# degleris1/CMF.jl

Hardware: NVIDIA B200
Metric: CNMF iterations/sec (higher is better)
Workload: dtype f32

## Files before the change

cmf.jl_b200/csrc/cmf_sm100.cu:

```cuda
#include "../../include/cmf_sm100.h"

#include <cuda_runtime.h>

#include <algorithm>
#include <chrono>
#include <cmath>
#include <cstdio>
#include <cstring>
#include <map>
#include <memory>
#include <mutex>
#include <tuple>
#include <stdexcept>
#include <string>
#include <vector>

#include <type_traits>

#include "kernels_simt.cuh"
#include "kernels_tc.cuh"
#include "kernels_fd.cuh"
#include "kernels_hals.cuh"
#include "comm.h"

namespace {

thread_local std::string g_err;

struct CmfError : std::runtime_error {
    int code;
    CmfError(int c, const std::string &m) : std::runtime_error(m), code(c) {}
};

#define CK(call)                                                                                   \
    do {                                                                                           \
        cudaError_t e__ = (call);                                                                  \
        if (e__ != cudaSuccess)                                                                    \
            throw CmfError(CMF_ERR_CUDA, std::string(#call) + ": " + cudaGetErrorString(e__));     \
    } while (0)

#define REQUIRE(cond, msg)                                                                         \
    do {                                                                                           \
        if (!(cond)) throw CmfError(CMF_ERR_ARG, std::string(msg));                                \
    } while (0)

inline int64_t cdiv(int64_t a, int64_t b) { return (a + b - 1) / b; }

template <typename T>
struct DevBuf {
    T *p = nullptr;
    size_t n = 0;
    DevBuf() = default;
    DevBuf(const DevBuf &) = delete;
    DevBuf &operator=(const DevBuf &) = delete;
    void alloc(size_t count) {
        free();
        n = count;
        if (count) {
            CK(cudaMalloc(&p, count * sizeof(T)));
            CK(cudaMemsetAsync(p, 0, count * sizeof(T), cudaStreamLegacy));
            CK(cudaStreamSynchronize(cudaStreamLegacy));
        }
    }
    void free() {
        if (p) cudaFree(p);
        p = nullptr;
        n = 0;
    }
    ~DevBuf() { free(); }
};

}

struct cmf_ctx {
    int64_t N = 0, T = 0, t0 = 0, t1 = 0, Tl = 0, K = 0, L = 0;
    int dtype = 0, alg = 0, device = 0, engine = 0;
    bool is_first = true, is_last = true;
    cudaStream_t stream = nullptr;
    bool own_stream = false;
    int64_t launches = 0;
    double data_norm = 0.0;
    double data_sumsq_local = 0.0;
    double data_sumsq_global = 0.0;
    int loss_mode = 0;
    bool loss_mode_explicit = false;
    double loss_guard = 0.25;
    int calib_max_interval = 16;
    bool calib_have = false;
    double calib_bias = 0.0, calib_last_err = 0.0;
    int calib_left = 0, calib_interval = 1, calib_fail = 0;
    int64_t n_loss_direct = 0, n_loss_expansion = 0;
    void calib_reset() { calib_have = false; calib_left = 0; calib_interval = 1; calib_fail = 0; numH_dot_valid = false; }
    double pgd_stepW = 5.0, pgd_stepH = 5.0, pgd_cur_loss = 0.0;
    bool numH_valid = false;
    bool numH_dot_valid = false;
    bool gram_valid = false;
    bool have_data = false, have_factors = false;
    int64_t R = 0;
    bool profiling = false;
    struct ProfEv { int which; cudaEvent_t a, b; };
    std::vector<ProfEv> prof_events;
    int prof_open = -1;
    void prof_begin(int which) {
        if (!profiling) return;
        ProfEv e; e.which = which;
        cudaEventCreate(&e.a); cudaEventCreate(&e.b);
        cudaEventRecord(e.a, stream);
        prof_events.push_back(e);
        prof_open = (int)prof_events.size() - 1;
    }
    void prof_end() {
        if (!profiling || prof_open < 0) return;
        cudaEventRecord(prof_events[prof_open].b, stream);
        prof_open = -1;
    }
    void prof_clear() {
        for (auto &e : prof_events) { cudaEventDestroy(e.a); cudaEventDestroy(e.b); }
        prof_events.clear();
    }
    virtual ~cmf_ctx() {
        prof_clear();
        if (ev_a) cudaEventDestroy(ev_a);
        if (ev_b) cudaEventDestroy(ev_b);
        if (comm_stream) cudaStreamDestroy(comm_stream);
    }
    cmf::Comm comm;
    cudaStream_t comm_stream = nullptr;
    cudaEvent_t ev_a = nullptr, ev_b = nullptr;
    struct cmf_multi *multi = nullptr;
    int world() const { return comm.world; }
    int rank() const { return comm.rank; }
    [[noreturn]] static void no_multi() { throw std::runtime_error("this call is not available on a multi-GPU group handle"); }
    virtual void get_data(void *, int) { no_multi(); }
    virtual bool tc_available() { no_multi(); }
    virtual bool fd_available() { no_multi(); }
    virtual void fd_release() { no_multi(); }
    virtual void set_data(const void *, int64_t) { no_multi(); }
    virtual void synth_data(uint64_t, int64_t, int64_t, double, double) { no_multi(); }
    virtual double data_sumsq() { no_multi(); }
    virtual void set_factors(const void *, const void *, int64_t) { no_multi(); }
    virtual void init_rand(uint64_t) { no_multi(); }
    virtual void init_scale_partials(double *) { no_multi(); }
    virtual void scale_factors(double) { no_multi(); }
    virtual void get_factors(void *, void *) { no_multi(); }
    virtual void w_partials() { no_multi(); }
    virtual void w_apply(double, double) { no_multi(); }
    virtual void w_denom_rows(int64_t, int64_t) { no_multi(); }
    virtual void w_update_rows(double, double, int64_t, int64_t) { no_multi(); }
    virtual void w_rows_buffers(void **, void **, int64_t *) { no_multi(); }
    virtual void fd_denomH_prefetch() {}
    virtual void h_update(double, double) { no_multi(); }
    virtual double loss_partial() { no_multi(); }
    virtual int loss_partial_dev() { no_multi(); }
    virtual double *scalars() { no_multi(); }
    virtual void hals_update_motifs(double, double) { no_multi(); }
    virtual double hals_update_feature_maps(double, double) { no_multi(); }
    virtual void hals_h_prepare() { no_multi(); }
    virtual void hals_h_local(void **, void **, int64_t *) { no_multi(); }
    virtual void hals_h_full(void **, void **) { no_multi(); }
    virtual void hals_h_sweep(int full, double, double) { no_multi(); }
    virtual void h_changed() { no_multi(); }
    virtual void fd_layout(int *, int *, int64_t *) { no_multi(); }
    virtual void set_pgd_loss(int, const void *) { no_multi(); }
    virtual void set_pgd_constraints(int, int) { no_multi(); }
    virtual void pgd_update_motifs(double, double) { no_multi(); }
    virtual double pgd_update_feature_maps(double, double) { no_multi(); }
    virtual void exchange_buffer(int, void **, int64_t *, int *) { no_multi(); }
    virtual void halo_buffers(void **, void **, void **, void **, int64_t *) { no_multi(); }
    virtual void prim_conv(void *) { no_multi(); }
    virtual void prim_transconv(const void *, void *) { no_multi(); }
    virtual void prim_corr(const void *, void *) { no_multi(); }
    virtual void prim_resids(void *) { no_multi(); }
    virtual void prim_shift_and_stack(void *) { no_multi(); }
    virtual void batch_set_factors(const void *, const void *) { no_multi(); }
    virtual void batch_get_factors(void *, void *) { no_multi(); }
    virtual void batch_scale_partials(double *) { no_multi(); }
    virtual void batch_scale(const double *) { no_multi(); }
    virtual void batch_loss(double *) { no_multi(); }
    virtual void batch_set_state(const double *, const int *) { no_multi(); }
    virtual void batch_update_motifs() { no_multi(); }
    virtual void batch_update_feature_maps() { no_multi(); }
};

enum { PROF_CONV = 0, PROF_TRANSCONV = 1, PROF_CORR = 2, PROF_SWEEP = 3, PROF_NCLASS = 4 };

namespace {

using namespace cmf;


typedef CUresult (*EncodeTiledFn)(CUtensorMap *, CUtensorMapDataType, cuuint32_t, void *, const cuuint64_t *,
                                  const cuuint64_t *, const cuuint32_t *, const cuuint32_t *, CUtensorMapInterleave,
                                  CUtensorMapSwizzle, CUtensorMapL2promotion, CUtensorMapFloatOOBfill);

EncodeTiledFn encode_tiled_fn() {
    static EncodeTiledFn fn = nullptr;
    if (!fn) {
        void *ptr = nullptr;
        cudaDriverEntryPointQueryResult qres;
        CK(cudaGetDriverEntryPoint("cuTensorMapEncodeTiled", &ptr, cudaEnableDefault, &qres));
        if (qres != cudaDriverEntryPointSuccess || !ptr) throw CmfError(CMF_ERR_CUDA, "cuTensorMapEncodeTiled not available");
        fn = (EncodeTiledFn)ptr;
    }
    return fn;
}

CUtensorMap make_map_2d(void *base, uint64_t dim0, uint64_t dim1, uint64_t stride1, uint32_t box0, uint32_t box1,
                        CUtensorMapSwizzle swz) {
    CUtensorMap m;
    cuuint64_t gdim[2] = {dim0, dim1};
    cuuint64_t gstr[1] = {stride1};
    cuuint32_t box[2] = {box0, box1};
    cuuint32_t estr[2] = {1, 1};
    CUresult r = encode_tiled_fn()(&m, CU_TENSOR_MAP_DATA_TYPE_BFLOAT16, 2, base, gdim, gstr, box, estr,
                                   CU_TENSOR_MAP_INTERLEAVE_NONE, swz, CU_TENSOR_MAP_L2_PROMOTION_L2_256B,
                                   CU_TENSOR_MAP_FLOAT_OOB_FILL_NONE);
    if (r != CUDA_SUCCESS) throw CmfError(CMF_ERR_CUDA, "cuTensorMapEncodeTiled failed with code " + std::to_string((int)r));
    return m;
}

CUtensorMap make_map_mn(void *base, uint64_t rows, uint64_t row_stride, uint64_t groups, uint32_t box_rows, uint32_t box_groups) {
    CUtensorMap m;
    cuuint64_t gdim[3] = {64, rows, groups};
    cuuint64_t gstr[2] = {row_stride, 128};
    cuuint32_t box[3] = {64, box_rows, box_groups};
    cuuint32_t estr[3] = {1, 1, 1};
    CUresult r = encode_tiled_fn()(&m, CU_TENSOR_MAP_DATA_TYPE_BFLOAT16, 3, base, gdim, gstr, box, estr,
                                   CU_TENSOR_MAP_INTERLEAVE_NONE, CU_TENSOR_MAP_SWIZZLE_128B, CU_TENSOR_MAP_L2_PROMOTION_L2_256B,
                                   CU_TENSOR_MAP_FLOAT_OOB_FILL_NONE);
    if (r != CUDA_SUCCESS) throw CmfError(CMF_ERR_CUDA, "cuTensorMapEncodeTiled (3-D) failed with code " + std::to_string((int)r));
    return m;
}

struct TcState {
    bool ok = false, tried = false;
    int Kp = 0, G = 0, num_sms = 148;
    int64_t KLp = 0, rows_u = 0, groups = 0, hrows = 0;
    DevBuf<__nv_bfloat16> X_hi, X_lo, Hw_hi, Hw_lo, Hm_hi, Hm_lo, Wc_hi, Wc_lo, Wu_hi, Wu_lo, Cc_hi, Cc_lo;
    CUtensorMap mWc[2], mHw[2], mHm[2], mWu[2], mXk[2], mXmn[2];
    CUtensorMap mHmn[2];
    CUtensorMap mCu[2];
    CUtensorMap mHk[2];
    CUtensorMap mGc[2];
    CUtensorMap mWuB[2], mWcB[2];
    DevBuf<__nv_bfloat16> Gc_hi, Gc_lo;
    int nsplit = 1, nsplit_g = 1;
    int64_t split_len = 0, split_len_g = 0, tiles_m = 0, tiles_n = 0, groups_c = 0, rows_c = 0;
    bool x_dirty = true, w_dirty = true;
};

struct FdState {
    bool ok = false, tried = false;
    int B = 0, logB = 0, V = 0, F = 0;
    int64_t nblk = 0, nblkp = 0;
    int Kq = 64, MR = 128;
    int V2 = 0;
    int64_t nblk2 = 0;
    DevBuf<__nv_bfloat16> Xf_hi, Xf_lo, Ah_hi, Ah_lo, Aw_hi, Aw_lo, Hf_hi, Hf_lo, Ac_hi, Ac_lo;
    DevBuf<float> Of, Df, Gf, Yf;
    DevBuf<__nv_bfloat16> Awm_hi, Awm_lo;
    int64_t nbc = 0;
    bool wx_dirty = true;
    CUtensorMap mXfK[2], mXfMN[2], mAw[2], mAh[2], mHfMN[2], mAc[2], mHf2K[2], mAwm[2], mHcK[2];
    bool x_dirty = true, w_dirty = true, h_dirty = true;
    bool hf2_valid = false;
    std::string why;
    void release() {
        Xf_hi.free(); Xf_lo.free(); Ah_hi.free(); Ah_lo.free(); Aw_hi.free(); Aw_lo.free(); Of.free(); Df.free();
        Hf_hi.free(); Hf_lo.free(); Gf.free(); Ac_hi.free(); Ac_lo.free();
        Yf.free(); Awm_hi.free(); Awm_lo.free(); nbc = 0; wx_dirty = true;
        ok = tried = false;
        x_dirty = w_dirty = h_dirty = true; hf2_valid = false;
    }
};

template <typename S>
struct Ctx : cmf_ctx {
    TcState tcs;
    FdState fds;
    DevBuf<S> X, Hbuf, Wi, Wtmp, numW, denW, GS, Cf, numH, denH, tailC;
    DevBuf<int> progress, lockstep;
    DevBuf<S> tailCt;
    int hals_grid = 0;
    DevBuf<double> exch1, corr_part, loss_part, scal;
    S *H = nullptr;
    int nsplit_w = 1, nsplit_g = 1;
    int64_t split_w = 0, split_g = 0;
    int conv_blocks_max = 0;

    static constexpr int TN = sizeof(S) == 4 ? 8 : 4;
    static constexpr int TT = 8, TY = 16;
    static constexpr int BN = 16 * TN, BT = TY * TT;

    int64_t KL() const { return K * L; }

    void hals_setup() {
        REQUIRE(L - 1 <= HW_TC, "HALS: L-1 must not exceed the sweep chunk (1024 columns)");
        const size_t smem = hals_wave_smem_elems<S>(L) * sizeof(S);
        int per_sm = 0, sms = 0, coop = 0;
        CK(cudaDeviceGetAttribute(&sms, cudaDevAttrMultiProcessorCount, device));
        CK(cudaDeviceGetAttribute(&coop, cudaDevAttrCooperativeLaunch, device));
        REQUIRE(coop != 0, "HALS needs cooperative launch support");
        CK(cudaFuncSetAttribute(hals_h_wave_kernel<S>, cudaFuncAttributeMaxDynamicSharedMemorySize, (int)smem));
        CK(cudaOccupancyMaxActiveBlocksPerMultiprocessor(&per_sm, hals_h_wave_kernel<S>, HW_NT, smem));
        hals_grid = (int)std::min<int64_t>(K, (int64_t)per_sm * sms);
        REQUIRE(hals_grid >= 1, "HALS: H sweep kernel does not fit on the device");
        tailC.alloc((size_t)hals_grid * (size_t)(L * L));
        progress.alloc((size_t)K);
    }

    void init() {
        if (R > 0) { init_batch(); return; }
        CK(cudaSetDevice(device));
        CK(cudaStreamCreateWithFlags(&stream, cudaStreamNonBlocking));
        own_stream = true;
        const int64_t hal = L - 1;
        X.alloc((size_t)((Tl + hal) * N));
        Hbuf.alloc((size_t)((Tl + 2 * hal) * K));
        H = Hbuf.p + hal * K;
        Wi.alloc((size_t)(KL() * N));
        Wtmp.alloc((size_t)(KL() * N));
        numW.alloc((size_t)(KL() * N));
        denW.alloc((size_t)(KL() * N));
        GS.alloc((size_t)(KL() * KL()));
        Cf.alloc((size_t)((2 * L - 1) * K * K));
        numH.alloc((size_t)(Tl * K));
        denH.alloc((size_t)(std::max<int64_t>(Tl * K, Tl)));
        exch1.alloc((size_t)(L * K * K + hal * K + 1));
        scal.alloc(8);
        if (alg == CMF_HALS) hals_setup();
        plan_split(N, Tl + hal, nsplit_w, split_w);
        plan_split(K, Tl + hal, nsplit_g, split_g);
        corr_part.alloc((size_t)std::max<int64_t>((int64_t)nsplit_w * KL() * N, (int64_t)nsplit_g * KL() * K));
        conv_blocks_max = (int)(cdiv(N, BN) * cdiv(Tl + hal, BT));
        loss_part.alloc((size_t)std::max(2 * conv_blocks_max, 4096));
        if (sizeof(S) == 4 && N >= 256 && Tl >= 4096 && K * L >= 256) {
            tc_setup();
            const char *e = getenv("CMF_ENGINE_DEFAULT");
            if (tcs.ok && engine == 1 && L >= 8 && K <= fd::KQ_MAX && !(e && atoi(e) == 1)) {
                fd_setup();
                if (fds.ok) { engine = 2; loss_mode = 1; }
            }
        }
        CK(cudaStreamSynchronize(stream));
    }

    bool tc_active() const { return engine >= 1 && tcs.ok; }
    bool fd_active() const { return engine == 2 && tcs.ok && fds.ok; }
    bool fd_available() override {
        if (!tc_available()) return false;
        if (!fds.ok && !fds.tried) fd_setup();
        if (fds.ok) { tcs.X_hi.free(); tcs.X_lo.free(); tcs.x_dirty = true; }
        return fds.ok;
    }
    void fd_release() override { fds.release(); }
    void fd_layout(int *B, int *V, int64_t *nblk) override {
        *B = fd_active() ? fds.B : 0; *V = fd_active() ? fds.V : 0; *nblk = fd_active() ? fds.nblkp : 0;
    }
    void mark_w_dirty() { tcs.w_dirty = true; fds.w_dirty = true; fds.wx_dirty = true; }

    void fd_setup() {
        if constexpr (!std::is_same<S, float>::value) { return; } else {
            FdState &f = fds;
            f.tried = true;
            if (!tcs.ok) { f.why = "needs the tcgen05 engine"; return; }
            if (K > fd::KQ_MAX || L > 256 || N < 16) { f.why = "needs K <= 128, L <= 256, N >= 16"; return; }
            f.Kq = (K <= 64) ? 64 : 128;
            f.MR = 2 * f.Kq;
            int B0 = 64;
            while (B0 < 8 * L && B0 < 1024) B0 *= 2;
            while (B0 < 4 * L) B0 *= 2;
            if (B0 / 2 >= 4 * L && B0 / 2 >= 64) {
                auto work = [&](int B) {
                    const int64_t nb = cdiv(Tl, (int64_t)(B - (int)L + 1));
                    return (double)(B / 2 + 1) * (double)(cdiv(nb, tc::BN) * tc::BN + cdiv(nb, 16) * 16);
                };
                if (work(B0) > 0.97 * work(B0 / 2)) B0 /= 2;
            }
            int forced = 0;
            if (const char *e = getenv("CMF_FD_B")) {
                const int want = atoi(e);
                if (want >= 4 * L && want >= 64 && want <= 1024 && (want & (want - 1)) == 0) forced = want;
            }
            tcs.X_hi.free(); tcs.X_lo.free(); tcs.x_dirty = true;
            size_t free_b = 0, total_b = 0;
            CK(cudaMemGetInfo(&free_b, &total_b));
            size_t later = (size_t)1 << 30;
            if (alg == CMF_HALS) later += (size_t)2 * (size_t)(Tl + 2048) * (size_t)K * 4 + (size_t)hals2::RING * (size_t)cdiv(K, hals2::GS) * (size_t)K * hals2::CW * 4;
            size_t xf = 0, ah = 0, aw = 0, of = 0, df = 0, hf = 0, gf = 0, ac = 0;
            bool fits = false;
            for (int B = forced ? forced : B0; B <= (forced ? forced : std::min(2 * B0, 1024)); B *= 2) {
                int logB = 0;
                while ((1 << logB) < B) ++logB;
                f.B = B; f.logB = logB; f.V = B - (int)L + 1; f.F = B / 2 + 1;
                f.nblk = cdiv(Tl, f.V);
                f.nblkp = cdiv(f.nblk, 16) * 16;
                xf = (size_t)f.F * (size_t)f.nblkp * 2 * (size_t)N + 64;
                ah = (size_t)f.F * (size_t)f.nblkp * 2 * f.MR + 64;
                aw = (size_t)f.F * f.MR * 2 * (size_t)N + 64;
                f.V2 = B - 2 * (int)L + 2;
                f.nblk2 = cdiv(Tl, f.V2);
                of = (size_t)f.F * (size_t)std::max(f.nblkp, f.nblk2) * f.MR; df = (size_t)f.F * f.MR * (size_t)N;
                hf = (size_t)f.F * (size_t)std::max(f.nblkp, f.nblk2) * 2 * f.Kq + 256; gf = (size_t)f.F * f.MR * f.Kq;
                ac = (size_t)f.F * f.MR * f.MR;
                const size_t need = 4 * (xf + ah + aw + hf + ac) + 4 * (of + df + gf);
                const size_t loss_pass = 4 * aw + (size_t)256 * (size_t)f.F * 2 * (size_t)N * sizeof(float);
                if (need + later + loss_pass <= free_b) { fits = true; break; }
            }
            if (!fits) { f.why = "not enough device memory for the spectrum of X"; return; }
            f.Xf_hi.alloc(xf); f.Xf_lo.alloc(xf);
            f.Ah_hi.alloc(ah); f.Ah_lo.alloc(ah);
            f.Aw_hi.alloc(aw); f.Aw_lo.alloc(aw);
            f.Of.alloc(of); f.Df.alloc(df);
            f.Hf_hi.alloc(hf); f.Hf_lo.alloc(hf); f.Gf.alloc(gf);
            f.Ac_hi.alloc(ac); f.Ac_lo.alloc(ac);
            __nv_bfloat16 *xs[2] = {f.Xf_hi.p, f.Xf_lo.p}, *as[2] = {f.Ah_hi.p, f.Ah_lo.p}, *ws[2] = {f.Aw_hi.p, f.Aw_lo.p};
            const uint64_t rows = (uint64_t)f.F * (uint64_t)f.nblkp;
            for (int i = 0; i < 2; ++i) {
                f.mXfK[i] = make_map_2d(xs[i], (uint64_t)(2 * N), rows, (uint64_t)N * 4, tc::BK, tc::BN, CU_TENSOR_MAP_SWIZZLE_64B);
                f.mXfMN[i] = make_map_mn(xs[i], rows * 2, (uint64_t)N * 2, (uint64_t)cdiv(N, 64), tc::BK, 4);
                f.mAw[i] = make_map_2d(ws[i], (uint64_t)(2 * N), (uint64_t)f.F * f.MR, (uint64_t)N * 4, tc::BK, tc::BM, CU_TENSOR_MAP_SWIZZLE_64B);
                f.mAh[i] = make_map_mn(as[i], rows * 2, (uint64_t)f.MR * 2, (uint64_t)(f.MR / 64), tc::BK, 2);
                f.mHfMN[i] = make_map_mn(i == 0 ? f.Hf_hi.p : f.Hf_lo.p, rows * 2, (uint64_t)f.Kq * 2, (uint64_t)(f.Kq / 64), tc::BK, 4);
                f.mAc[i] = make_map_2d(i == 0 ? f.Ac_hi.p : f.Ac_lo.p, f.MR, (uint64_t)f.F * f.MR, (uint64_t)f.MR * 2, tc::BK, tc::BM, CU_TENSOR_MAP_SWIZZLE_64B);
                f.mHf2K[i] = make_map_2d(i == 0 ? f.Hf_hi.p : f.Hf_lo.p, f.MR, (uint64_t)f.F * (uint64_t)f.nblk2, (uint64_t)f.MR * 2, tc::BK, tc::BN, CU_TENSOR_MAP_SWIZZLE_64B);
            }
            CK(cudaFuncSetAttribute(tc::tc_kernel<tc::TC_FQT>, cudaFuncAttributeMaxDynamicSharedMemorySize, tc::SMEM_BYTES));
            CK(cudaFuncSetAttribute(tc::tc_kernel<tc::TC_FQC>, cudaFuncAttributeMaxDynamicSharedMemorySize, tc::SMEM_BYTES));
            CK(cudaFuncSetAttribute(tc::tc_kernel<tc::TC_FQX>, cudaFuncAttributeMaxDynamicSharedMemorySize, tc::SMEM_BYTES));

            const int big = (int)fd_smem(fd_cols_h()), small_ = (int)fd_smem(16);
            CK(cudaFuncSetAttribute(fd::fft_x_kernel, cudaFuncAttributeMaxDynamicSharedMemorySize, small_));
            CK(cudaFuncSetAttribute(fd::ifft_resid_kernel, cudaFuncAttributeMaxDynamicSharedMemorySize, small_));
            CK(cudaFuncSetAttribute(fd::fft_w_kernel, cudaFuncAttributeMaxDynamicSharedMemorySize, small_));
            CK(cudaFuncSetAttribute(fd::ifft_numW_kernel<float>, cudaFuncAttributeMaxDynamicSharedMemorySize, small_));
            CK(cudaFuncSetAttribute(fd::ifft_numW_kernel<double>, cudaFuncAttributeMaxDynamicSharedMemorySize, small_));
            CK(cudaFuncSetAttribute(fd::fft_h_kernel, cudaFuncAttributeMaxDynamicSharedMemorySize, big));
            CK(cudaFuncSetAttribute(fd::ifft_numH_kernel, cudaFuncAttributeMaxDynamicSharedMemorySize, big));
            f.x_dirty = f.w_dirty = f.h_dirty = true;
            f.ok = true;
        }
    }
    int fd_cols_h() const {
        if (const char *e = getenv("CMF_FD_COLS")) {
            const int c = atoi(e);
            if ((c == 8 || c == 16 || c == 32) && (size_t)fds.B * (size_t)c * sizeof(float2) <= 160 * 1024) return c;
        }
        return fds.B >= 1024 ? 8 : 16;
    }
    int64_t fd_order(int64_t nblocks) const { static const int o = getenv("CMF_FD_ORDER") ? atoi(getenv("CMF_FD_ORDER")) : 0; return o ? nblocks : 0; }
    int fd_cols_w() const { return fds.B >= 1024 ? 8 : 16; }
    size_t fd_smem(int C) const { return ((size_t)fds.B * (size_t)C + (size_t)fds.B) * sizeof(float2); }

    void fd_build_X() {
        if constexpr (std::is_same<S, float>::value) {
            FdState &f = fds;
            if (!f.x_dirty) return;
            dim3 grid((unsigned)(f.nblkp * cdiv(N, 32)));
            fd::fft_x_kernel<<<grid, fd::NT, fd_smem(16), stream>>>(X.p, f.Xf_hi.p, f.Xf_lo.p, N, Tl + (L - 1), f.B, f.logB, f.V, f.nblkp, fd_order(f.nblkp));
            post_launch();
            f.x_dirty = false;
        }
    }
    void fd_corr() {
        if constexpr (std::is_same<S, float>::value) {
            FdState &f = fds;
            fd_build_X();
            fd_spectrum_H();
            tc::Params q = tc_base_params();
            q.nprod = 3;
            q.tiles_n = cdiv(N, tc::BN);
            q.nkb = f.nblkp * 2 / tc::BK;
            q.MR = f.MR; q.mtiles = f.MR / tc::BM; q.units = (int64_t)f.F * q.tiles_n * q.mtiles;
            q.fq_rows = f.nblkp * 2;
            q.out = f.Df.p; q.Mrows = f.MR; q.Ncols = N; q.ldo = N;
            const unsigned grid = (unsigned)std::min<int64_t>(q.units, tcs.num_sms);
            prof_begin(PROF_CORR);
            tc::tc_kernel<tc::TC_FQC><<<grid, tc::THREADS, tc::SMEM_BYTES, stream>>>(f.mAh[0], f.mAh[1], f.mXfMN[0], f.mXfMN[1], q);
            prof_end();
            post_launch();
            fd::ifft_numW_kernel<float><<<dim3((unsigned)cdiv(N, 2 * fd_cols_w()), (unsigned)K), fd::NT, fd_smem(fd_cols_w()), stream>>>(f.Df.p, numW.p, N, N, K, L, f.B, f.logB, f.Kq, fd_cols_w());
            post_launch();
        }
    }
    void fd_denomH() {
        if constexpr (std::is_same<S, float>::value) {
            FdState &f = fds;
            fd::fft_w_kernel<<<dim3((unsigned)cdiv(K, 2 * fd_cols_w()), (unsigned)K), fd::NT, fd_smem(fd_cols_w()), stream>>>(
                Cf.p, f.Ac_hi.p, f.Ac_lo.p, K, K, 2 * L - 1, f.B, f.logB, f.MR, f.Kq, 0, f.Kq, fd_cols_w());
            post_launch();
            const int C = fd_cols_h();
            fd_denomH_prefetch();
            f.hf2_valid = false;
            tc::Params q = tc_base_params();
            q.nprod = 3;
            q.tiles_n = cdiv(f.nblk2, tc::BN);
            q.nkb = f.MR / tc::BK;
            q.MR = f.MR; q.mtiles = f.MR / tc::BM; q.units = (int64_t)f.F * q.tiles_n * q.mtiles;
            q.fq_rows = f.nblk2;
            q.out = f.Of.p;
            const unsigned grid = (unsigned)std::min<int64_t>(q.units, tcs.num_sms);
            tc::tc_kernel<tc::TC_FQT><<<grid, tc::THREADS, tc::SMEM_BYTES, stream>>>(f.mAc[0], f.mAc[1], f.mHf2K[0], f.mHf2K[1], q);
            post_launch();
            fd::ifft_numH_kernel<<<(unsigned)(f.nblk2 * (f.Kq / 2 / C)), fd::NT, fd_smem(C), stream>>>(
                f.Of.p, denH.p, K, Tl, f.B, f.logB, f.V2, f.nblk2, C, f.Kq, fd_order(f.nblk2));
            post_launch();
        }
    }
    void fd_denomH_prefetch() override {
        if constexpr (std::is_same<S, float>::value) {
            FdState &f = fds;
            if (!fd_active() || f.hf2_valid) return;
            const int C = fd_cols_h();
            fd::fft_h_kernel<<<(unsigned)(f.nblk2 * (f.Kq / 2 / C)), fd::NT, fd_smem(C), stream>>>(
                H, f.Hf_hi.p, f.Hf_lo.p, K, Tl, Tl + (L - 1), f.B, f.logB, f.V2, f.nblk2, C, 1, -(L - 1), f.Kq, fd_order(f.nblk2));
            post_launch();
            f.hf2_valid = true;
        }
    }
    int64_t fd_conv_loss() {
        if constexpr (std::is_same<S, float>::value) {
            FdState &f = fds;
            f.hf2_valid = false;
            const int64_t ntile32 = cdiv(N, 32);
            if (f.Awm_hi.n == 0) {
                const size_t aw = (size_t)f.F * 2 * f.MR * (size_t)N + 64;
                size_t free_b = 0, total_b = 0;
                CK(cudaMemGetInfo(&free_b, &total_b));
                const size_t per_block = (size_t)f.F * 2 * (size_t)N * sizeof(float);
                REQUIRE(free_b > 4 * aw + 256 * per_block + ((size_t)1 << 29), "not enough device memory for the frequency-domain loss pass");
                size_t budget = std::min<size_t>((free_b - 4 * aw - ((size_t)1 << 29)) / 2, (size_t)12 << 30);
                int64_t nbc = (int64_t)(budget / per_block) / tc::BN * tc::BN;
                nbc = std::max<int64_t>(tc::BN, std::min<int64_t>(nbc, cdiv(f.nblk, tc::BN) * tc::BN));
                if (const char *e = getenv("CMF_FD_NBC")) { const int64_t v = atoll(e); if (v >= tc::BN && v % tc::BN == 0 && v < nbc) nbc = v; }
                f.nbc = nbc;
                f.Awm_hi.alloc(aw); f.Awm_lo.alloc(aw);
                f.Yf.alloc((size_t)f.F * (size_t)nbc * 2 * (size_t)N);
                for (int i = 0; i < 2; ++i) {
                    f.mAwm[i] = make_map_mn(i == 0 ? f.Awm_hi.p : f.Awm_lo.p, (uint64_t)f.F * 2 * f.MR, (uint64_t)N * 2, (uint64_t)cdiv(N, 64), tc::BK, 2);
                    f.mHcK[i] = make_map_2d(i == 0 ? f.Hf_hi.p : f.Hf_lo.p, f.MR, (uint64_t)f.F * (uint64_t)f.nblk, (uint64_t)f.MR * 2, tc::BK, tc::BN, CU_TENSOR_MAP_SWIZZLE_64B);
                }
                f.wx_dirty = true;
            }
            const size_t need_lp = (size_t)(f.nblk * ntile32);
            if (loss_part.n < need_lp) loss_part.alloc(std::max<size_t>(need_lp, 4096));
            if (f.wx_dirty) {
                fd::fft_w_kernel<<<dim3((unsigned)cdiv(N, 2 * fd_cols_w()), (unsigned)K), fd::NT, fd_smem(fd_cols_w()), stream>>>(Wi.p, f.Awm_hi.p, f.Awm_lo.p, N, K, L, f.B, f.logB, 2 * N, N, 1, f.Kq, fd_cols_w());
                post_launch();
                f.wx_dirty = false;
            }
            const int C = fd_cols_h();
            fd::fft_h_kernel<<<(unsigned)(f.nblk * (f.Kq / 2 / C)), fd::NT, fd_smem(C), stream>>>(
                H, f.Hf_hi.p, f.Hf_lo.p, K, Tl, Tl + (L - 1), f.B, f.logB, f.V, f.nblk, C, 1, -(L - 1), f.Kq, fd_order(f.nblk));
            post_launch();
            prof_begin(PROF_CONV);
            for (int64_t b0 = 0; b0 < f.nblk; b0 += f.nbc) {
                const int64_t cur = std::min(f.nbc, f.nblk - b0);
                tc::Params q = tc_base_params();
                q.nprod = 3;
                q.tiles_n = cdiv(cur, tc::BN);
                q.tiles_m = cdiv(N, tc::BM);
                q.nkb = f.MR / tc::BK;
                q.MR = f.MR; q.mtiles = 1; q.units = (int64_t)f.F * 2 * q.tiles_m * q.tiles_n;
                q.fq_rows = f.nblk; q.b_off = b0; q.nbc = cur;
                q.out = f.Yf.p;
                const unsigned grid = (unsigned)std::min<int64_t>(q.units, tcs.num_sms);
                tc::tc_kernel<tc::TC_FQX><<<grid, tc::THREADS, tc::SMEM_BYTES, stream>>>(f.mAwm[0], f.mAwm[1], f.mHcK[0], f.mHcK[1], q);
                post_launch();
                fd::ifft_resid_kernel<<<(unsigned)(cur * ntile32), fd::NT, fd_smem(16), stream>>>(
                    f.Yf.p, X.p, loss_part.p + b0 * ntile32, N, Tl, L, f.B, f.logB, f.V, cur, b0, fd_order(cur));
                post_launch();
            }
            prof_end();
            return f.nblk * ntile32;
        }
        return 0;
    }
    void fd_spectrum_H() {
        if constexpr (std::is_same<S, float>::value) {
            FdState &f = fds;
            if (!f.h_dirty) return;
            const int C = fd_cols_h();
            fd::fft_h_kernel<<<(unsigned)(f.nblkp * (f.Kq / 2 / C)), fd::NT, fd_smem(C), stream>>>(
                H, f.Ah_hi.p, f.Ah_lo.p, K, Tl, Tl + (L - 1), f.B, f.logB, f.V, f.nblkp, C, 0, 0, f.Kq, fd_order(f.nblkp));
            post_launch();
            f.h_dirty = false;
        }
    }
    void fd_gram() {
        if constexpr (std::is_same<S, float>::value) {
            FdState &f = fds;
            f.hf2_valid = false;
            fd_spectrum_H();
            const int C = fd_cols_h();
            fd::fft_h_kernel<<<(unsigned)(f.nblkp * (f.Kq / 2 / C)), fd::NT, fd_smem(C), stream>>>(
                H, f.Hf_hi.p, f.Hf_lo.p, K, Tl, Tl + (L - 1), f.B, f.logB, f.V, f.nblkp, C, 1, 0, f.Kq, fd_order(f.nblkp));
            post_launch();
            tc::Params q = tc_base_params();
            q.nprod = 3;
            q.tiles_n = 1;
            q.nkb = f.nblkp * 2 / tc::BK;
            q.MR = f.MR; q.mtiles = f.MR / tc::BM; q.units = (int64_t)f.F * q.mtiles;
            q.fq_rows = f.nblkp * 2;
            q.out = f.Gf.p; q.Mrows = f.MR; q.Ncols = K; q.ldo = f.Kq;
            const unsigned grid = (unsigned)std::min<int64_t>(q.units, tcs.num_sms);
            tc::tc_kernel<tc::TC_FQC><<<grid, tc::THREADS, tc::SMEM_BYTES, stream>>>(f.mAh[0], f.mAh[1], f.mHfMN[0], f.mHfMN[1], q);
            post_launch();
            fd::ifft_numW_kernel<double><<<dim3((unsigned)cdiv(K, 2 * fd_cols_w()), (unsigned)K), fd::NT, fd_smem(fd_cols_w()), stream>>>(f.Gf.p, exch1.p, K, f.Kq, K, L, f.B, f.logB, f.Kq, fd_cols_w());
            post_launch();
        }
    }
    void fd_transconv() {
        if constexpr (std::is_same<S, float>::value) {
            FdState &f = fds;
            fd_build_X();
            if (f.w_dirty) {
                fd::fft_w_kernel<<<dim3((unsigned)cdiv(N, 2 * fd_cols_w()), (unsigned)K), fd::NT, fd_smem(fd_cols_w()), stream>>>(Wi.p, f.Aw_hi.p, f.Aw_lo.p, N, K, L, f.B, f.logB, 2 * N, N, 0, f.Kq, fd_cols_w());
                post_launch();
                f.w_dirty = false;
            }
            tc::Params q = tc_base_params();
            q.nprod = 3;
            q.tiles_n = cdiv(f.nblkp, tc::BN);
            q.nkb = cdiv(2 * N, tc::BK);
            q.MR = f.MR; q.mtiles = f.MR / tc::BM; q.units = (int64_t)f.F * q.tiles_n * q.mtiles;
            q.fq_rows = f.nblkp;
            q.out = f.Of.p;
            const unsigned grid = (unsigned)std::min<int64_t>(q.units, tcs.num_sms);
            prof_begin(PROF_TRANSCONV);
            tc::tc_kernel<tc::TC_FQT><<<grid, tc::THREADS, tc::SMEM_BYTES, stream>>>(f.mAw[0], f.mAw[1], f.mXfK[0], f.mXfK[1], q);
            prof_end();
            post_launch();
            const int C = fd_cols_h();
            fd::ifft_numH_kernel<<<(unsigned)(f.nblk * (f.Kq / 2 / C)), fd::NT, fd_smem(C), stream>>>(
                f.Of.p, numH.p, K, Tl, f.B, f.logB, f.V, f.nblkp, C, f.Kq, fd_order(f.nblk));
            post_launch();
        }
    }
    bool tc_available() override {
        if (!tcs.ok && !tcs.tried) tc_setup();
        return tcs.ok;
    }

    void tc_setup() {
        if constexpr (!std::is_same<S, float>::value) { return; } else {
            TcState &t = tcs;
            t.tried = true;
            if (K > 128 || N % 8 != 0) return;
            t.Kp = (int)(cdiv(K, 8) * 8);
            t.G = 128 / t.Kp;
            t.KLp = cdiv(L * t.Kp, 64) * 64;
            t.groups = cdiv(L, t.G);
            t.rows_u = cdiv(L * t.Kp + 128, 128) * 128;
            const int64_t hal = L - 1;
            t.hrows = Tl + hal;
            cudaDeviceProp prop;
            CK(cudaGetDeviceProperties(&prop, device));
            if (prop.major != 10) return;
            t.num_sms = prop.multiProcessorCount;
            t.Wc_hi.alloc((size_t)(N * t.KLp)); t.Wc_lo.alloc((size_t)(N * t.KLp));
            t.Wu_hi.alloc((size_t)(t.rows_u * N)); t.Wu_lo.alloc((size_t)(t.rows_u * N));
            t.groups_c = cdiv(2 * L - 1, t.G);
            t.rows_c = cdiv((2 * L - 1) * t.Kp + 128, 128) * 128;
            t.Cc_hi.alloc((size_t)(t.rows_c * t.Kp)); t.Cc_lo.alloc((size_t)(t.rows_c * t.Kp));
            t.Gc_hi.alloc((size_t)(KL() * t.KLp)); t.Gc_lo.alloc((size_t)(KL() * t.KLp));
            if (GS.n < (size_t)(t.rows_u * t.rows_u)) GS.alloc((size_t)(t.rows_u * t.rows_u));
            __nv_bfloat16 *wc[2] = {t.Wc_hi.p, t.Wc_lo.p};
            __nv_bfloat16 *wu[2] = {t.Wu_hi.p, t.Wu_lo.p};
            for (int i = 0; i < 2; ++i) {
                t.mWc[i] = make_map_2d(wc[i], (uint64_t)t.KLp, (uint64_t)N, (uint64_t)t.KLp * 2, tc::BK, tc::BM, CU_TENSOR_MAP_SWIZZLE_64B);
                t.mWu[i] = make_map_2d(wu[i], (uint64_t)N, (uint64_t)t.rows_u, (uint64_t)N * 2, tc::BK, tc::BM, CU_TENSOR_MAP_SWIZZLE_64B);
                __nv_bfloat16 *cc[2] = {t.Cc_hi.p, t.Cc_lo.p};
                t.mCu[i] = make_map_2d(cc[i], (uint64_t)t.Kp, (uint64_t)t.rows_c, (uint64_t)t.Kp * 2, tc::BK, tc::BM, CU_TENSOR_MAP_SWIZZLE_64B);
                __nv_bfloat16 *gc[2] = {t.Gc_hi.p, t.Gc_lo.p};
                t.mWuB[i] = make_map_2d(wu[i], (uint64_t)N, (uint64_t)t.rows_u, (uint64_t)N * 2, tc::BK, tc::BN, CU_TENSOR_MAP_SWIZZLE_64B);
                t.mWcB[i] = make_map_2d(wc[i], (uint64_t)t.KLp, (uint64_t)N, (uint64_t)t.KLp * 2, tc::BK, tc::BN, CU_TENSOR_MAP_SWIZZLE_64B);
                t.mGc[i] = make_map_2d(gc[i], (uint64_t)t.KLp, (uint64_t)KL(), (uint64_t)t.KLp * 2, tc::BK, tc::BM, CU_TENSOR_MAP_SWIZZLE_64B);
            }
            t.tiles_m = cdiv(t.KLp, tc::BM);
            t.tiles_n = cdiv(N, tc::BN);
            const int64_t tau = Tl + hal, base = t.tiles_m * t.tiles_n;
            double best = -1.0;
            for (int ns = 1; ns <= 16; ++ns) {
                const int64_t sl = cdiv(cdiv(tau, ns), tc::BK) * tc::BK;
                if (ns > 1 && sl < tc::FLUSH_T) break;
                const int64_t units = base * cdiv(tau, sl);
                const double eff = (double)units / (double)(cdiv(units, t.num_sms) * t.num_sms);
                if (eff > best + 1e-9) { best = eff; t.nsplit = (int)cdiv(tau, sl); t.split_len = sl; }
            }
            {
                const int64_t want = std::max<int64_t>(1, cdiv(2 * t.num_sms, t.tiles_m));
                const int64_t maxs = std::max<int64_t>(1, tau / tc::FLUSH_T);
                const int64_t ns = std::min(want, maxs);
                t.split_len_g = cdiv(cdiv(tau, ns), tc::BK) * tc::BK;
                t.nsplit_g = (int)cdiv(tau, t.split_len_g);
            }
            const size_t need = std::max((size_t)t.nsplit * (size_t)(KL() * N), (size_t)t.nsplit_g * (size_t)(KL() * K));
            if (corr_part.n < need) corr_part.alloc(need);
            const size_t need_lp = (size_t)(tc::EPI_WARPS * cdiv(Tl, tc::BN) * cdiv(N, tc::BM));
            if (loss_part.n < need_lp) loss_part.alloc(std::max<size_t>(need_lp, 4096));
            CK(cudaFuncSetAttribute(tc::tc_kernel<tc::TC_CONV>, cudaFuncAttributeMaxDynamicSharedMemorySize, tc::SMEM_BYTES));
            CK(cudaFuncSetAttribute(tc::tc_kernel<tc::TC_TRANS>, cudaFuncAttributeMaxDynamicSharedMemorySize, tc::SMEM_BYTES));
            CK(cudaFuncSetAttribute(tc::tc_kernel<tc::TC_CORR>, cudaFuncAttributeMaxDynamicSharedMemorySize, tc::SMEM_BYTES));
            CK(cudaFuncSetAttribute(tc::tc_kernel<tc::TC_PLAIN>, cudaFuncAttributeMaxDynamicSharedMemorySize, tc::SMEM_BYTES));
            t.ok = true;
            t.x_dirty = t.w_dirty = true;
            if (N >= 256 && Tl >= 4096 && K * L >= 256) engine = 1;
        }
    }

    tc::Params tc_base_params() {
        tc::Params q;
        memset(&q, 0, sizeof(q));
        q.N = N; q.K = K; q.L = L; q.Tl = Tl; q.G = tcs.G; q.Kp = tcs.Kp;
        { const char *e = getenv("CMF_PROMO"); q.promo = e ? std::max(1, atoi(e)) : tc::PROMO; }
        { const char *e = getenv("CMF_TC_PRODUCTS"); q.nprod = (e && atoi(e) == 2) ? 2 : 3; }
        return q;
    }

    void tc_split_X() {
        if constexpr (std::is_same<S, float>::value) {
            if (!tcs.ok || !tcs.x_dirty) return;
            TcState &t = tcs;
            if (t.X_hi.n == 0) {
                const int64_t hal = L - 1;
                t.X_hi.alloc(X.n + 64); t.X_lo.alloc(X.n + 64);
                __nv_bfloat16 *xs[2] = {t.X_hi.p, t.X_lo.p};
                for (int i = 0; i < 2; ++i) {
                    t.mXk[i] = make_map_2d(xs[i], (uint64_t)N, (uint64_t)(Tl + hal), (uint64_t)N * 2, tc::BK, tc::BN, CU_TENSOR_MAP_SWIZZLE_64B);
                    t.mXmn[i] = make_map_mn(xs[i], (uint64_t)(Tl + hal), (uint64_t)N * 2, (uint64_t)cdiv(N, 64), tc::BK, 4);
                }
            }
            tc::split_plain_kernel<<<(unsigned)cdiv((int64_t)X.n, 256), 256, 0, stream>>>(X.p, tcs.X_hi.p, tcs.X_lo.p, (int64_t)X.n);
            post_launch();
            tcs.x_dirty = false;
        }
    }
    void tc_split_W() {
        if constexpr (std::is_same<S, float>::value) {
            if (!tcs.w_dirty) return;
            tc::split_W_kernel<<<dim3((unsigned)cdiv(N, 32), (unsigned)cdiv(tcs.Kp, 32), (unsigned)L), dim3(32, 8), 0, stream>>>(
                Wi.p, tcs.Wc_hi.p, tcs.Wc_lo.p, tcs.Wu_hi.p, tcs.Wu_lo.p, N, K, L, tcs.Kp, tcs.KLp);
            post_launch();
            tcs.w_dirty = false;
        }
    }
    void tc_h_planes() {
        if constexpr (std::is_same<S, float>::value) {
            TcState &t = tcs;
            if (t.Hw_hi.n != 0) return;
            const int64_t hal = L - 1;
            const size_t hw_elems = (size_t)((Tl + 2 * hal) * t.Kp + t.KLp + 64);
            t.Hw_hi.alloc(hw_elems); t.Hw_lo.alloc(hw_elems);
            t.Hm_hi.alloc(hw_elems); t.Hm_lo.alloc(hw_elems);
            __nv_bfloat16 *hw[2] = {t.Hw_hi.p, t.Hw_lo.p}, *hm[2] = {t.Hm_hi.p, t.Hm_lo.p};
            for (int i = 0; i < 2; ++i) {
                t.mHw[i] = make_map_2d(hw[i], (uint64_t)t.KLp, (uint64_t)t.hrows, (uint64_t)t.Kp * 2, tc::BK, tc::BN, CU_TENSOR_MAP_SWIZZLE_64B);
                t.mHm[i] = make_map_mn(hm[i], (uint64_t)t.hrows, (uint64_t)t.Kp * 2, (uint64_t)(t.KLp / 64), tc::BK, 2);
                t.mHmn[i] = make_map_mn(hw[i] + hal * t.Kp, (uint64_t)(Tl + hal), (uint64_t)t.Kp * 2, (uint64_t)cdiv(t.Kp, 64), tc::BK, 4);
                t.mHk[i] = make_map_2d(hw[i], (uint64_t)t.Kp, (uint64_t)(Tl + 2 * hal), (uint64_t)t.Kp * 2, tc::BK, tc::BN, CU_TENSOR_MAP_SWIZZLE_64B);
            }
        }
    }
    void tc_split_H(bool masked) {
        if constexpr (std::is_same<S, float>::value) {
            tc_h_planes();
            const int64_t rows = Tl + 2 * (L - 1);
            tc::split_H_kernel<<<(unsigned)cdiv(rows * tcs.Kp, 256), 256, 0, stream>>>(
                Hbuf.p, masked ? tcs.Hm_hi.p : tcs.Hw_hi.p, masked ? tcs.Hm_lo.p : tcs.Hw_lo.p, rows, K, tcs.Kp,
                L - 1, L - 1 + Tl, masked ? 1 : 0);
            post_launch();
        }
    }

    void tc_corr() {
        if constexpr (std::is_same<S, float>::value) {
            if (fd_active()) { fd_corr(); return; }
            tc_split_X();
            tc_split_H(true);
            tc::Params q = tc_base_params();
            q.tiles_m = tcs.tiles_m; q.tiles_n = tcs.tiles_n; q.split_len = tcs.split_len; q.tau_hi = Tl + (L - 1);
            q.units = tcs.tiles_m * tcs.tiles_n * tcs.nsplit;
            q.part = corr_part.p;
            q.corr_order = 0;
            {
                const char *e = getenv("CMF_LOCKSTEP");
                const int w = e ? atoi(e) : 256;
                if (w > 0) {
                    if (lockstep.n == 0) lockstep.alloc(1024);
                    CK(cudaMemsetAsync(lockstep.p, 0, lockstep.n * sizeof(int), stream));
                    q.lockstep = lockstep.p; q.lockstep_window = w;
                }
            }
            const unsigned grid = (unsigned)std::min<int64_t>(q.units, tcs.num_sms);
            prof_begin(PROF_CORR);
            if (q.lockstep != nullptr) {
                void *args[] = {&tcs.mHm[0], &tcs.mHm[1], &tcs.mXmn[0], &tcs.mXmn[1], &q};
                CK(cudaLaunchCooperativeKernel((void *)tc::tc_kernel<tc::TC_CORR>, dim3(grid), dim3(tc::THREADS), args, tc::SMEM_BYTES, stream));
            } else {
                tc::tc_kernel<tc::TC_CORR><<<grid, tc::THREADS, tc::SMEM_BYTES, stream>>>(tcs.mHm[0], tcs.mHm[1], tcs.mXmn[0], tcs.mXmn[1], q);
            }
            prof_end();
            post_launch();
            const int64_t n = KL() * N;
            reduce_partials_kernel<S><<<(unsigned)cdiv(n, 256), 256, 0, stream>>>(corr_part.p, tcs.nsplit, n, numW.p, nullptr);
            post_launch();
        }
    }
    void tc_plain(const CUtensorMap *mA, const CUtensorMap *mB, S *out, int64_t Mrows, int64_t Ncols, int64_t Kdim, int64_t ldo, bool sym = false) {
        if constexpr (std::is_same<S, float>::value) {
            tc::Params q = tc_base_params();
            q.sym = (sym && !getenv("CMF_S2_FULL")) ? 1 : 0;
            q.tiles_n = cdiv(Ncols, tc::BN);
            q.nkb = cdiv(Kdim, tc::BK);
            q.units = q.tiles_n * cdiv(Mrows, tc::BM);
            q.out = out; q.Mrows = Mrows; q.Ncols = Ncols; q.ldo = ldo;
            const unsigned grid = (unsigned)std::min<int64_t>(q.units, tcs.num_sms);
            tc::tc_kernel<tc::TC_PLAIN><<<grid, tc::THREADS, tc::SMEM_BYTES, stream>>>(mA[0], mA[1], mB[0], mB[1], q);
            post_launch();
            if (q.sym) {
                tc::mirror_upper_kernel<<<dim3((unsigned)cdiv(Mrows, 256), (unsigned)Mrows), 256, 0, stream>>>(out, Mrows, ldo);
                post_launch();
            }
        }
    }
    void tc_denomW(int64_t j0 = 0, int64_t j1 = -1) {
        if (j1 < 0) j1 = KL();
        if constexpr (std::is_same<S, float>::value) {
            if (getenv("CMF_G_DIRECT"))
                tc::build_G_split_kernel<<<(unsigned)cdiv(KL() * tcs.KLp, 256), 256, 0, stream>>>(
                    exch1.p, exch1.p + L * K * K, tcs.Gc_hi.p, tcs.Gc_lo.p, K, L, tcs.Kp, tcs.KLp);
            else
                tc::build_G_split_diag_kernel<<<(unsigned)cdiv((2 * L - 1) * K * K, 256), 256, 0, stream>>>(
                    exch1.p, exch1.p + L * K * K, tcs.Gc_hi.p, tcs.Gc_lo.p, K, L, tcs.Kp, tcs.KLp);
            post_launch();
            tc_split_W();
            if (j0 == 0 && j1 == KL()) {
                tc_plain(tcs.mGc, tcs.mWcB, denW.p, KL(), N, tcs.KLp, N);
            } else {
                CUtensorMap mg[2];
                __nv_bfloat16 *gc[2] = {tcs.Gc_hi.p, tcs.Gc_lo.p};
                for (int i = 0; i < 2; ++i)
                    mg[i] = make_map_2d(gc[i] + j0 * tcs.KLp, (uint64_t)tcs.KLp, (uint64_t)(j1 - j0), (uint64_t)tcs.KLp * 2, tc::BK, tc::BM, CU_TENSOR_MAP_SWIZZLE_64B);
                tc_plain(mg, tcs.mWcB, denW.p + j0 * N, j1 - j0, N, tcs.KLp, N);
            }
        }
    }
    void tc_gram() {
        if constexpr (std::is_same<S, float>::value) {
            tc::Params q = tc_base_params();
            q.N = K;
            q.tiles_m = tcs.tiles_m; q.tiles_n = 1; q.split_len = tcs.split_len_g; q.tau_hi = Tl + (L - 1);
            q.units = tcs.tiles_m * tcs.nsplit_g;
            q.part = corr_part.p;
            const unsigned grid = (unsigned)std::min<int64_t>(q.units, tcs.num_sms);
            tc::tc_kernel<tc::TC_CORR><<<grid, tc::THREADS, tc::SMEM_BYTES, stream>>>(tcs.mHm[0], tcs.mHm[1], tcs.mHmn[0], tcs.mHmn[1], q);
            post_launch();
            const int64_t n = L * K * K;
            reduce_partials_kernel<S><<<(unsigned)cdiv(n, 256), 256, 0, stream>>>(corr_part.p, tcs.nsplit_g, n, nullptr, exch1.p);
            post_launch();
        }
    }
    void tc_denomH(bool resplit_C = true) {
        if constexpr (std::is_same<S, float>::value) {
            if (resplit_C) {
                tc::split_C_kernel<<<(unsigned)cdiv(tcs.rows_c * tcs.Kp, 256), 256, 0, stream>>>(Cf.p, tcs.Cc_hi.p, tcs.Cc_lo.p, K, 2 * L - 1, tcs.Kp, tcs.rows_c);
                post_launch();
            }
            tc::Params q = tc_base_params();
            q.groups = tcs.groups_c; q.nblocks = cdiv(tcs.Kp, tc::BK); q.own = tc::BN - (tcs.G - 1);
            q.units = cdiv(Tl, q.own);
            q.out = denH.p;
            const unsigned grid = (unsigned)std::min<int64_t>(q.units, tcs.num_sms);
            tc::tc_kernel<tc::TC_TRANS><<<grid, tc::THREADS, tc::SMEM_BYTES, stream>>>(tcs.mCu[0], tcs.mCu[1], tcs.mHk[0], tcs.mHk[1], q);
            post_launch();
        }
    }
    void tc_transconv() {
        if constexpr (std::is_same<S, float>::value) {
            if (fd_active()) { fd_transconv(); return; }
            tc_split_X();
            tc_split_W();
            tc::Params q = tc_base_params();
            q.groups = tcs.groups; q.nblocks = cdiv(N, tc::BK); q.own = tc::BN - (tcs.G - 1);
            q.units = cdiv(Tl, q.own);
            q.out = numH.p;
            const unsigned grid = (unsigned)std::min<int64_t>(q.units, tcs.num_sms);
            {
                const char *e = getenv("CMF_LOCKSTEP_TRANS");
                const int w = e ? atoi(e) : 0;
                if (w > 0 && q.units >= (int64_t)grid) {
                    if (lockstep.n == 0) lockstep.alloc(1024);
                    CK(cudaMemsetAsync(lockstep.p, 0, lockstep.n * sizeof(int), stream));
                    q.lockstep = lockstep.p; q.lockstep_window = w;
                }
            }
            prof_begin(PROF_TRANSCONV);
            if (q.lockstep != nullptr) {
                void *args[] = {&tcs.mWu[0], &tcs.mWu[1], &tcs.mXk[0], &tcs.mXk[1], &q};
                CK(cudaLaunchCooperativeKernel((void *)tc::tc_kernel<tc::TC_TRANS>, dim3(grid), dim3(tc::THREADS), args, tc::SMEM_BYTES, stream));
            } else {
                tc::tc_kernel<tc::TC_TRANS><<<grid, tc::THREADS, tc::SMEM_BYTES, stream>>>(tcs.mWu[0], tcs.mWu[1], tcs.mXk[0], tcs.mXk[1], q);
            }
            prof_end();
            post_launch();
        }
    }
    int64_t tc_conv_loss() {
        if constexpr (std::is_same<S, float>::value) {
            tc_split_W();
            tc_split_H(false);
            tc::Params q = tc_base_params();
            q.tiles_n = cdiv(N, tc::BM);
            q.nkb = tcs.KLp / tc::BK;
            q.units = q.tiles_n * cdiv(Tl, tc::BN);
            q.X = X.p; q.partial = loss_part.p;
            const unsigned grid = (unsigned)std::min<int64_t>(q.units, tcs.num_sms);
            prof_begin(PROF_CONV);
            tc::tc_kernel<tc::TC_CONV><<<grid, tc::THREADS, tc::SMEM_BYTES, stream>>>(tcs.mWc[0], tcs.mWc[1], tcs.mHw[0], tcs.mHw[1], q);
            prof_end();
            post_launch();
            return tc::EPI_WARPS * q.units;
        }
        return 0;
    }

    ~Ctx() override {
        if (tracing) trace_dump();
        if (own_stream && stream) cudaStreamDestroy(stream);
    }

    void plan_split(int64_t Nin, int64_t tau_hi, int &nsplit, int64_t &split_len, int64_t Kc = 0, int64_t nrest = 1) {
        const int64_t ngrp = cdiv(L, 8);
        const int64_t bxy = cdiv(Nin, 128) * cdiv((Kc ? Kc : K) * ngrp, CORR_PB) * nrest;
        int64_t ns = std::min<int64_t>(std::max<int64_t>(cdiv(592, bxy), 1), 64);
        split_len = cdiv(cdiv(tau_hi, ns), CORR_BTAU) * CORR_BTAU;
        if (split_len < CORR_BTAU) split_len = CORR_BTAU;
        nsplit = (int)cdiv(tau_hi, split_len);
// ... 1855 lines not shown
```

cmf.jl_b200/csrc/kernels_fd.cuh:

```cuda
#pragma once
#include <cuda_bf16.h>
#include <cuda_runtime.h>
#include <stdint.h>

namespace cmf {
namespace fd {

#ifndef CMF_FD_MINB
#define CMF_FD_MINB 3
#endif
constexpr int LD_U = 8;
constexpr int NT = 512;
constexpr int KQ_MAX = 128;

__device__ __forceinline__ void make_twiddles(float2 *tw, int B) {
    for (int m = threadIdx.x; m < B; m += NT) {
        float s, c;
        sincospif(-2.0f * (float)m / (float)B, &s, &c);
        tw[m] = make_float2(c, s);
    }
}

__device__ __forceinline__ int rev(int x, int logB) { return (int)(__brev((unsigned)x) >> (32 - logB)); }

__device__ __forceinline__ float2 cmul(float2 a, float2 w) { return make_float2(a.x * w.x - a.y * w.y, a.x * w.y + a.y * w.x); }
__device__ __forceinline__ float2 cadd(float2 a, float2 b) { return make_float2(a.x + b.x, a.y + b.y); }
__device__ __forceinline__ float2 csub(float2 a, float2 b) { return make_float2(a.x - b.x, a.y - b.y); }
template <bool INV> __device__ __forceinline__ float2 mul_mi(float2 a) { return INV ? make_float2(-a.y, a.x) : make_float2(a.y, -a.x); }
template <bool INV> __device__ __forceinline__ float2 mul_w8(float2 a) {
    const float r = 0.70710678118654752f;
    return INV ? make_float2((a.x - a.y) * r, (a.x + a.y) * r) : make_float2((a.x + a.y) * r, (a.y - a.x) * r);
}
template <bool INV> __device__ __forceinline__ float2 mul_w83(float2 a) {
    const float r = 0.70710678118654752f;
    return INV ? make_float2((-a.x - a.y) * r, (a.x - a.y) * r) : make_float2((a.y - a.x) * r, (-a.x - a.y) * r);
}

template <bool INV>
__device__ __forceinline__ void fft_passes(float2 *d, const float2 *tw, int B, int logB, int C) {
    const int c = threadIdx.x % C, j0 = threadIdx.x / C, jstep = NT / C;
    int s = 0;
    for (; s + 2 < logB; s += 3) {
        const int lq = logB - s - 3, q = 1 << lq, qC = q * C;
        for (int j = j0; j < (B >> 3); j += jstep) {
            const int pos = j & (q - 1), g = j >> lq;
            float2 *r = d + ((g << (lq + 3)) + pos) * C + c;
            float2 a0 = r[0], a1 = r[qC], a2 = r[2 * qC], a3 = r[3 * qC], a4 = r[4 * qC], a5 = r[5 * qC], a6 = r[6 * qC], a7 = r[7 * qC];
            float2 t;
            t = csub(a0, a4); a0 = cadd(a0, a4); a4 = t;
            t = csub(a1, a5); a1 = cadd(a1, a5); a5 = mul_w8<INV>(t);
            t = csub(a2, a6); a2 = cadd(a2, a6); a6 = mul_mi<INV>(t);
            t = csub(a3, a7); a3 = cadd(a3, a7); a7 = mul_w83<INV>(t);
            t = csub(a0, a2); a0 = cadd(a0, a2); a2 = t;
            t = csub(a1, a3); a1 = cadd(a1, a3); a3 = mul_mi<INV>(t);
            t = csub(a4, a6); a4 = cadd(a4, a6); a6 = t;
            t = csub(a5, a7); a5 = cadd(a5, a7); a7 = mul_mi<INV>(t);
            t = csub(a0, a1); a0 = cadd(a0, a1); a1 = t;
            t = csub(a2, a3); a2 = cadd(a2, a3); a3 = t;
            t = csub(a4, a5); a4 = cadd(a4, a5); a5 = t;
            t = csub(a6, a7); a6 = cadd(a6, a7); a7 = t;
            if (lq > 0) {
                const int e = pos << s;
                float2 w;
#define CMF_TW(m_, a_) w = tw[(m_) * e]; if (INV) w.y = -w.y; a_ = cmul(a_, w);
                CMF_TW(4, a1) CMF_TW(2, a2) CMF_TW(6, a3) CMF_TW(1, a4) CMF_TW(5, a5) CMF_TW(3, a6) CMF_TW(7, a7)
#undef CMF_TW
            }
            r[0] = a0; r[qC] = a1; r[2 * qC] = a2; r[3 * qC] = a3; r[4 * qC] = a4; r[5 * qC] = a5; r[6 * qC] = a6; r[7 * qC] = a7;
        }
        __syncthreads();
    }
    if (logB - s == 2) {
        for (int j = j0; j < (B >> 2); j += jstep) {
            float2 *r = d + (4 * j) * C + c;
            float2 a0 = r[0], a1 = r[C], a2 = r[2 * C], a3 = r[3 * C], t;
            t = csub(a0, a2); a0 = cadd(a0, a2); a2 = t;
            t = csub(a1, a3); a1 = cadd(a1, a3); a3 = mul_mi<INV>(t);
            r[0] = cadd(a0, a1); r[C] = csub(a0, a1); r[2 * C] = cadd(a2, a3); r[3 * C] = csub(a2, a3);
        }
        __syncthreads();
    } else if (logB - s == 1) {
        for (int j = j0; j < (B >> 1); j += jstep) {
            float2 *r0 = d + (2 * j) * C + c, *r1 = r0 + C;
            const float2 a = *r0, b = *r1;
            *r0 = cadd(a, b);
            *r1 = csub(a, b);
        }
        __syncthreads();
    }
}

__device__ __forceinline__ void unpack_pair(const float2 *d, int f, int B, int logB, int C, int p, float &ar, float &ai, float &br,
                                            float &bi) {
    const float2 z = d[rev(f, logB) * C + p], y = d[rev((B - f) & (B - 1), logB) * C + p];
    ar = 0.5f * (z.x + y.x); ai = 0.5f * (z.y - y.y);
    br = 0.5f * (z.y + y.y); bi = -0.5f * (z.x - y.x);
}

__device__ __forceinline__ void pack_pair(float2 *d, int f, int B, int C, int p, float2 re, float2 im) {
    if (f == 0 || f == B / 2) im = make_float2(0.f, 0.f);
    d[f * C + p] = make_float2(re.x - im.y, im.x + re.y);
    if (f > 0 && f < B / 2) d[(B - f) * C + p] = make_float2(re.x + im.y, re.y - im.x);
}

__device__ __forceinline__ void split2(float a, float b, uint32_t &h, uint32_t &l) {
    const __nv_bfloat162 hh = __floats2bfloat162_rn(a, b);
    const float2 hf = __bfloat1622float2(hh);
    const __nv_bfloat162 ll = __floats2bfloat162_rn(a - hf.x, b - hf.y);
    h = *reinterpret_cast<const uint32_t *>(&hh);
    l = *reinterpret_cast<const uint32_t *>(&ll);
}
__device__ __forceinline__ void store_split2(__nv_bfloat16 *hi, __nv_bfloat16 *lo, int64_t idx, float a, float b) {
    uint32_t h, l;
    split2(a, b, h, l);
    *reinterpret_cast<uint32_t *>(hi + idx) = h;
    *reinterpret_cast<uint32_t *>(lo + idx) = l;
}

__global__ void __launch_bounds__(NT, CMF_FD_MINB)
fft_x_kernel(const float *__restrict__ X, __nv_bfloat16 *__restrict__ hi, __nv_bfloat16 *__restrict__ lo, int64_t N, int64_t xcols,
             int B, int logB, int V, int64_t nblkp, int64_t nbx) {
    extern __shared__ float2 fd_smem[];
    constexpr int C = 16;
    float2 *d = fd_smem, *tw = fd_smem + (size_t)B * C;
    const int ny = (int)((N + 31) / 32);
    const int64_t b = nbx ? blockIdx.x % nbx : blockIdx.x / ny;
    const int p = threadIdx.x % C;
    const int64_t n = (int64_t)(nbx ? blockIdx.x / nbx : blockIdx.x % ny) * 32 + 2 * p;
    make_twiddles(tw, B);
    {
        const int i0 = threadIdx.x / C, istep = NT / C;
        const int64_t lim64 = xcols - b * V;
        const int lim = (n < N) ? (int)(lim64 < 0 ? 0 : (lim64 > B ? B : lim64)) : 0;
        const float *src = X + (b * V + i0) * N + n;
        for (int i = i0; i < B; i += LD_U * istep, src += (int64_t)LD_U * istep * N) {
            float2 v[LD_U];
#pragma unroll
            for (int u = 0; u < LD_U; ++u) {
                v[u] = make_float2(0.f, 0.f);
                if (i + u * istep < lim) v[u] = *reinterpret_cast<const float2 *>(src + (int64_t)u * istep * N);
            }
#pragma unroll
            for (int u = 0; u < LD_U; ++u)
                if (i + u * istep < B) d[(i + u * istep) * C + p] = v[u];
        }
    }
    __syncthreads();
    fft_passes<false>(d, tw, B, logB, C);
    if (n >= N) return;
    for (int f = threadIdx.x / C; f <= B / 2; f += NT / C) {
        float ar, ai, br, bi;
        unpack_pair(d, f, B, logB, C, p, ar, ai, br, bi);
        const int64_t r = ((int64_t)f * nblkp + b) * 2;
        store_split2(hi, lo, r * N + n, ar, br);
        store_split2(hi, lo, (r + 1) * N + n, ai, bi);
    }
}

__global__ void __launch_bounds__(NT, CMF_FD_MINB)
fft_h_kernel(const float *__restrict__ H, __nv_bfloat16 *__restrict__ hi, __nv_bfloat16 *__restrict__ lo, int64_t K, int64_t Tl,
             int64_t hcols, int B, int logB, int V, int64_t nblkp, int C, int full, int64_t t_off, int kq, int64_t nbx) {
    const int64_t KQ = kq, MROWS = 2 * kq;
    extern __shared__ float2 fd_smem[];
    float2 *d = fd_smem, *tw = fd_smem + (size_t)B * C;
    const int ny = (kq / 2) / C;
    const int64_t b = nbx ? blockIdx.x % nbx : blockIdx.x / ny;
    const int p = threadIdx.x % C;
    const int k = 2 * ((int)(nbx ? blockIdx.x / nbx : blockIdx.x % ny) * C + p);
    make_twiddles(tw, B);
    {
        const int i0 = threadIdx.x / C, istep = NT / C;
        const int64_t tb = b * V + t_off;
        const int64_t lim64 = full ? (hcols - tb) : ((Tl - tb < V) ? Tl - tb : V);
        const int lim = (int)(lim64 < 0 ? 0 : (lim64 > B ? B : lim64));
        const float *src = H + (tb + i0) * K + k;
        const bool pair = ((K & 1) == 0) && (k + 1 < K);
        for (int i = i0; i < B; i += LD_U * istep, src += (int64_t)LD_U * istep * K) {
            float2 v[LD_U];
#pragma unroll
            for (int u = 0; u < LD_U; ++u) {
                v[u] = make_float2(0.f, 0.f);
                if (i + u * istep < lim) {
                    const float *q = src + (int64_t)u * istep * K;
                    if (pair) v[u] = *reinterpret_cast<const float2 *>(q);
                    else { if (k < K) v[u].x = q[0]; if (k + 1 < K) v[u].y = q[1]; }
                }
            }
#pragma unroll
            for (int u = 0; u < LD_U; ++u)
                if (i + u * istep < B) d[(i + u * istep) * C + p] = v[u];
        }
    }
    __syncthreads();
    fft_passes<false>(d, tw, B, logB, C);
    for (int f = threadIdx.x / C; f <= B / 2; f += NT / C) {
        float ar, ai, br, bi;
        unpack_pair(d, f, B, logB, C, p, ar, ai, br, bi);
        uint32_t hr, lr, hi_, li_;
        split2(ar, br, hr, lr);
        split2(ai, bi, hi_, li_);
        if (full) {
            const int64_t r = (((int64_t)f * nblkp + b) * 2) * KQ + k;
            *reinterpret_cast<uint32_t *>(hi + r) = hr; *reinterpret_cast<uint32_t *>(lo + r) = lr;
            *reinterpret_cast<uint32_t *>(hi + r + KQ) = hi_; *reinterpret_cast<uint32_t *>(lo + r + KQ) = li_;
            continue;
        }
        const int64_t r = (((int64_t)f * nblkp + b) * 2) * MROWS + k;
        const uint32_t sg = 0x80008000u;
        *reinterpret_cast<uint32_t *>(hi + r) = hr; *reinterpret_cast<uint32_t *>(lo + r) = lr;
        *reinterpret_cast<uint32_t *>(hi + r + KQ) = hi_ ^ sg; *reinterpret_cast<uint32_t *>(lo + r + KQ) = li_ ^ sg;
        *reinterpret_cast<uint32_t *>(hi + r + MROWS) = hi_; *reinterpret_cast<uint32_t *>(lo + r + MROWS) = li_;
        *reinterpret_cast<uint32_t *>(hi + r + MROWS + KQ) = hr; *reinterpret_cast<uint32_t *>(lo + r + MROWS + KQ) = lr;
    }
}

__global__ void __launch_bounds__(NT, CMF_FD_MINB)
fft_w_kernel(const float *__restrict__ Wi, __nv_bfloat16 *__restrict__ hi, __nv_bfloat16 *__restrict__ lo, int64_t N, int64_t K,
             int64_t L, int B, int logB, int64_t ldw, int64_t coff, int xmode, int kq, int C) {
    const int64_t KQ = kq, MROWS = 2 * kq;
    extern __shared__ float2 fd_smem[];
    float2 *d = fd_smem, *tw = fd_smem + (size_t)B * C;
    const int64_t k = blockIdx.y;
    const int p = threadIdx.x % C;
    const int64_t n = (int64_t)blockIdx.x * (2 * C) + 2 * p;
    make_twiddles(tw, B);
    {
        const int i0 = threadIdx.x / C, istep = NT / C;
        for (int i = i0; i < B; i += LD_U * istep) {
            float2 v[LD_U];
#pragma unroll
            for (int u = 0; u < LD_U; ++u) {
                const int ii = i + u * istep;
                v[u] = make_float2(0.f, 0.f);
                if (ii < L && n < N) {
                    const float *src = Wi + ((int64_t)ii * K + k) * N + n;
                    if ((N & 1) == 0) v[u] = *reinterpret_cast<const float2 *>(src);
                    else { v[u].x = src[0]; if (n + 1 < N) v[u].y = src[1]; }
                }
            }
#pragma unroll
            for (int u = 0; u < LD_U; ++u)
                if (i + u * istep < B) d[(i + u * istep) * C + p] = v[u];
        }
    }
    __syncthreads();
    fft_passes<false>(d, tw, B, logB, C);
    if (n >= N) return;
    for (int f = threadIdx.x / C; f <= B / 2; f += NT / C) {
        float ar, ai, br, bi;
        unpack_pair(d, f, B, logB, C, p, ar, ai, br, bi);
        if (xmode) {
            const int64_t r0 = (((int64_t)f * 2 + 0) * MROWS + k) * N + n, r1 = (((int64_t)f * 2 + 1) * MROWS + k) * N + n;
            store_split2(hi, lo, r0, ar, br);
            store_split2(hi, lo, r0 + KQ * N, -ai, -bi);
            store_split2(hi, lo, r1, ai, bi);
            store_split2(hi, lo, r1 + KQ * N, ar, br);
            continue;
        }
        const int64_t re = ((int64_t)f * MROWS + k) * ldw, im = ((int64_t)f * MROWS + KQ + k) * ldw;
        store_split2(hi, lo, re + n, ar, br);
        store_split2(hi, lo, re + coff + n, ai, bi);
        store_split2(hi, lo, im + n, -ai, -bi);
        store_split2(hi, lo, im + coff + n, ar, br);
    }
}

__global__ void __launch_bounds__(NT, CMF_FD_MINB)
ifft_numH_kernel(const float *__restrict__ Of, float *__restrict__ numH, int64_t K, int64_t Tl, int B, int logB, int V,
                 int64_t nblkp, int C, int kq, int64_t nbx) {
    const int64_t KQ = kq, MROWS = 2 * kq;
    extern __shared__ float2 fd_smem[];
    float2 *d = fd_smem, *tw = fd_smem + (size_t)B * C;
    const int ny = (kq / 2) / C;
    const int64_t b = nbx ? blockIdx.x % nbx : blockIdx.x / ny;
    const int p = threadIdx.x % C;
    const int k = 2 * ((int)(nbx ? blockIdx.x / nbx : blockIdx.x % ny) * C + p);
    make_twiddles(tw, B);
    {
        const int f0 = threadIdx.x / C, fstep = NT / C;
        const float *o = Of + ((int64_t)f0 * nblkp + b) * MROWS + k;
        for (int f = f0; f <= B / 2; f += 4 * fstep, o += (int64_t)4 * fstep * nblkp * MROWS) {
            float2 re[4], im[4];
#pragma unroll
            for (int u = 0; u < 4; ++u)
                if (f + u * fstep <= B / 2) {
                    const float *q = o + (int64_t)u * fstep * nblkp * MROWS;
                    re[u] = *reinterpret_cast<const float2 *>(q); im[u] = *reinterpret_cast<const float2 *>(q + KQ);
                }
#pragma unroll
            for (int u = 0; u < 4; ++u)
                if (f + u * fstep <= B / 2) pack_pair(d, f + u * fstep, B, C, p, re[u], im[u]);
        }
    }
    __syncthreads();
    fft_passes<true>(d, tw, B, logB, C);
    const float sc = 1.0f / (float)B;
    const bool pair = ((K & 1) == 0) && (k + 1 < K);
    for (int i = threadIdx.x / C; i < V; i += NT / C) {
        const int64_t t = b * V + i;
        if (t >= Tl) break;
        const float2 z = d[rev(i, logB) * C + p];
        if (pair) *reinterpret_cast<float2 *>(numH + t * K + k) = make_float2(z.x * sc, z.y * sc);
        else { if (k < K) numH[t * K + k] = z.x * sc; if (k + 1 < K) numH[t * K + k + 1] = z.y * sc; }
    }
}

__global__ void __launch_bounds__(NT, CMF_FD_MINB)
ifft_resid_kernel(const float *__restrict__ Yf, const float *__restrict__ X, double *__restrict__ partial, int64_t N, int64_t Tl,
                  int64_t L, int B, int logB, int V, int64_t nbc, int64_t b0, int64_t nbx) {
    extern __shared__ float2 fd_smem[];
    __shared__ double red[NT / 32];
    constexpr int C = 16;
    float2 *d = fd_smem, *tw = fd_smem + (size_t)B * C;
    const int ny = (int)((N + 31) / 32);
    const int64_t bc = nbx ? blockIdx.x % nbx : blockIdx.x / ny;
    const int by = (int)(nbx ? blockIdx.x / nbx : blockIdx.x % ny);
    const int p = threadIdx.x % C;
    const int64_t n = (int64_t)by * 32 + 2 * p;
    make_twiddles(tw, B);
    {
        const int f0 = threadIdx.x / C, fstep = NT / C;
        const float *y = Yf + (((int64_t)f0 * nbc + bc) * 2) * N + n;
        for (int f = f0; f <= B / 2; f += 4 * fstep, y += (int64_t)4 * fstep * nbc * 2 * N) {
            float2 re[4], im[4];
#pragma unroll
            for (int u = 0; u < 4; ++u) {
                re[u] = make_float2(0.f, 0.f); im[u] = re[u];
                if (f + u * fstep <= B / 2 && n < N) {
                    const float *q = y + (int64_t)u * fstep * nbc * 2 * N;
                    re[u] = *reinterpret_cast<const float2 *>(q); im[u] = *reinterpret_cast<const float2 *>(q + N);
                }
            }
#pragma unroll
            for (int u = 0; u < 4; ++u)
                if (f + u * fstep <= B / 2) pack_pair(d, f + u * fstep, B, C, p, re[u], im[u]);
        }
    }
    __syncthreads();
    fft_passes<true>(d, tw, B, logB, C);
    const float sc = 1.0f / (float)B;
    double accd = 0.0;
    if (n < N) {
        const int istep = NT / C;
        const int64_t tb = (b0 + bc) * V - (L - 1);
        for (int i = (int)(L - 1) + threadIdx.x / C; i < B; i += LD_U * istep) {
            float2 x[LD_U];
#pragma unroll
            for (int u = 0; u < LD_U; ++u) {
                const int ii = i + u * istep;
                x[u] = make_float2(0.f, 0.f);
                if (ii < B && tb + ii < Tl) x[u] = *reinterpret_cast<const float2 *>(X + (tb + ii) * N + n);
            }
            float acc = 0.f;
#pragma unroll
            for (int u = 0; u < LD_U; ++u) {
                const int ii = i + u * istep;
                if (ii < B && tb + ii < Tl) {
                    const float2 z = d[rev(ii, logB) * C + p];
                    const float r0 = z.x * sc - x[u].x, r1 = z.y * sc - x[u].y;
                    acc = fmaf(r0, r0, acc);
                    acc = fmaf(r1, r1, acc);
                }
            }
            accd += (double)acc;
        }
    }
#pragma unroll
    for (int o = 16; o > 0; o >>= 1) accd += __shfl_xor_sync(0xffffffffu, accd, o);
    if ((threadIdx.x & 31) == 0) red[threadIdx.x >> 5] = accd;
    __syncthreads();
    if (threadIdx.x == 0) {
        double s = 0.0;
        for (int w = 0; w < NT / 32; ++w) s += red[w];
        partial[bc * ny + by] = s;
    }
}

template <typename OutT>
__global__ void __launch_bounds__(NT, CMF_FD_MINB)
ifft_numW_kernel(const float *__restrict__ Df, OutT *__restrict__ out, int64_t N, int64_t ldi, int64_t K, int64_t L, int B, int logB,
                 int kq, int C) {
    const int64_t KQ = kq, MROWS = 2 * kq;
    extern __shared__ float2 fd_smem[];
    float2 *d = fd_smem, *tw = fd_smem + (size_t)B * C;
    const int64_t k = blockIdx.y;
    const int p = threadIdx.x % C;
    const int64_t n = (int64_t)blockIdx.x * (2 * C) + 2 * p;
    make_twiddles(tw, B);
    {
        const int f0 = threadIdx.x / C, fstep = NT / C;
        for (int f = f0; f <= B / 2; f += 4 * fstep) {
            float2 re[4], im[4];
#pragma unroll
            for (int u = 0; u < 4; ++u) {
                const int ff = f + u * fstep;
                re[u] = make_float2(0.f, 0.f); im[u] = re[u];
                if (ff <= B / 2 && n < N) {
                    re[u] = *reinterpret_cast<const float2 *>(Df + ((int64_t)ff * MROWS + k) * ldi + n);
                    im[u] = *reinterpret_cast<const float2 *>(Df + ((int64_t)ff * MROWS + KQ + k) * ldi + n);
                }
            }
#pragma unroll
            for (int u = 0; u < 4; ++u)
                if (f + u * fstep <= B / 2) pack_pair(d, f + u * fstep, B, C, p, re[u], im[u]);
        }
    }
    __syncthreads();
    fft_passes<true>(d, tw, B, logB, C);
    if (n >= N) return;
    const float sc = 1.0f / (float)B;
    for (int l = threadIdx.x / C; l < L; l += NT / C) {
        const float2 z = d[rev(l, logB) * C + p];
        OutT *o = out + ((int64_t)l * K + k) * N + n;
        if (sizeof(OutT) == 4) {
            *reinterpret_cast<float2 *>(o) = make_float2(z.x * sc, z.y * sc);
        } else {
            o[0] = (OutT)(z.x * sc);
            if (n + 1 < N) o[1] = (OutT)(z.y * sc);
        }
    }
}

}
}
```

Measured before the change: 23.23.

## Template FFT kernels on block length and width, precompute twiddles, use packed float2 math

The frequency-domain FFT kernels become templates on log block length and tile width, so loop bounds, strides and bit-reversal are compile-time constants and loops can be fully unrolled. Twiddle factors are computed once into a device buffer and copied into shared memory, instead of each block evaluating sincospif. The butterfly and scaling arithmetic uses packed float2 intrinsics (__fadd2_rn, __ffma2_rn). In exchange there are many more kernel instantiations, and block lengths outside 64–1024 are rejected.

After: 24.98, median of 6. +7.5%, better.

```diff
diff --git a/cmf.jl_b200/csrc/cmf_sm100.cu b/cmf.jl_b200/csrc/cmf_sm100.cu
--- a/cmf.jl_b200/csrc/cmf_sm100.cu
+++ b/cmf.jl_b200/csrc/cmf_sm100.cu
@@ -258,6 +258,7 @@
     int64_t nblk2 = 0;
     DevBuf<__nv_bfloat16> Xf_hi, Xf_lo, Ah_hi, Ah_lo, Aw_hi, Aw_lo, Hf_hi, Hf_lo, Ac_hi, Ac_lo;
     DevBuf<float> Of, Df, Gf, Yf;
+    DevBuf<float2> tw;
     DevBuf<__nv_bfloat16> Awm_hi, Awm_lo;
     int64_t nbc = 0;
     bool wx_dirty = true;
@@ -267,12 +268,35 @@
     std::string why;
     void release() {
         Xf_hi.free(); Xf_lo.free(); Ah_hi.free(); Ah_lo.free(); Aw_hi.free(); Aw_lo.free(); Of.free(); Df.free();
-        Hf_hi.free(); Hf_lo.free(); Gf.free(); Ac_hi.free(); Ac_lo.free();
+        Hf_hi.free(); Hf_lo.free(); Gf.free(); Ac_hi.free(); Ac_lo.free(); tw.free();
         Yf.free(); Awm_hi.free(); Awm_lo.free(); nbc = 0; wx_dirty = true;
         ok = tried = false;
         x_dirty = w_dirty = h_dirty = true; hf2_valid = false;
     }
 };
+
+template <typename Fn>
+void fd_with_b(int logB, Fn &&fn) {
+    switch (logB) {
+    case 6: fn(std::integral_constant<int, 6>{}); break;
+    case 7: fn(std::integral_constant<int, 7>{}); break;
+    case 8: fn(std::integral_constant<int, 8>{}); break;
+    case 9: fn(std::integral_constant<int, 9>{}); break;
+    case 10: fn(std::integral_constant<int, 10>{}); break;
+    default: REQUIRE(false, "frequency-domain transforms: block length must be a power of two in [64, 1024]");
+    }
+}
+template <typename Fn>
+void fd_with_bc(int logB, int C, Fn &&fn) {
+    fd_with_b(logB, [&](auto lb) {
+        switch (C) {
+        case 8: fn(lb, std::integral_constant<int, 8>{}); break;
+        case 16: fn(lb, std::integral_constant<int, 16>{}); break;
+        case 32: fn(lb, std::integral_constant<int, 32>{}); break;
+        default: REQUIRE(false, "frequency-domain transforms: unsupported tile width");
+        }
+    });
+}
 
 template <typename S>
 struct Ctx : cmf_ctx {
@@ -414,6 +438,9 @@
             f.Of.alloc(of); f.Df.alloc(df);
             f.Hf_hi.alloc(hf); f.Hf_lo.alloc(hf); f.Gf.alloc(gf);
             f.Ac_hi.alloc(ac); f.Ac_lo.alloc(ac);
+            f.tw.alloc((size_t)f.B);
+            fd::twiddle_kernel<<<(unsigned)cdiv(f.B, 256), 256, 0, stream>>>(f.tw.p, f.B);
+            post_launch();
             __nv_bfloat16 *xs[2] = {f.Xf_hi.p, f.Xf_lo.p}, *as[2] = {f.Ah_hi.p, f.Ah_lo.p}, *ws[2] = {f.Aw_hi.p, f.Aw_lo.p};
             const uint64_t rows = (uint64_t)f.F * (uint64_t)f.nblkp;
             for (int i = 0; i < 2; ++i) {
@@ -429,14 +456,27 @@
             CK(cudaFuncSetAttribute(tc::tc_kernel<tc::TC_FQC>, cudaFuncAttributeMaxDynamicSharedMemorySize, tc::SMEM_BYTES));
             CK(cudaFuncSetAttribute(tc::tc_kernel<tc::TC_FQX>, cudaFuncAttributeMaxDynamicSharedMemorySize, tc::SMEM_BYTES));
 
-            const int big = (int)fd_smem(fd_cols_h()), small_ = (int)fd_smem(16);
-            CK(cudaFuncSetAttribute(fd::fft_x_kernel, cudaFuncAttributeMaxDynamicSharedMemorySize, small_));
-            CK(cudaFuncSetAttribute(fd::ifft_resid_kernel, cudaFuncAttributeMaxDynamicSharedMemorySize, small_));
-            CK(cudaFuncSetAttribute(fd::fft_w_kernel, cudaFuncAttributeMaxDynamicSharedMemorySize, small_));
-            CK(cudaFuncSetAttribute(fd::ifft_numW_kernel<float>, cudaFuncAttributeMaxDynamicSharedMemorySize, small_));
-            CK(cudaFuncSetAttribute(fd::ifft_numW_kernel<double>, cudaFuncAttributeMaxDynamicSharedMemorySize, small_));
-            CK(cudaFuncSetAttribute(fd::fft_h_kernel, cudaFuncAttributeMaxDynamicSharedMemorySize, big));
-            CK(cudaFuncSetAttribute(fd::ifft_numH_kernel, cudaFuncAttributeMaxDynamicSharedMemorySize, big));
+            fd_with_b(f.logB, [&](auto lb) {
+                constexpr int LB = decltype(lb)::value;
+                const int x16 = (int)fd_smem(16), w = (int)fd_smem(fd_cols_w());
+                CK(cudaFuncSetAttribute(fd::fft_x_kernel<LB>, cudaFuncAttributeMaxDynamicSharedMemorySize, x16));
+                CK(cudaFuncSetAttribute(fd::ifft_resid_kernel<LB>, cudaFuncAttributeMaxDynamicSharedMemorySize, x16));
+                fd_with_bc(f.logB, fd_cols_w(), [&](auto, auto c) {
+                    constexpr int CW = decltype(c)::value;
+                    CK(cudaFuncSetAttribute(fd::fft_w_kernel<LB, CW>, cudaFuncAttributeMaxDynamicSharedMemorySize, w));
+                    CK(cudaFuncSetAttribute(fd::ifft_numW_kernel<float, LB, CW>, cudaFuncAttributeMaxDynamicSharedMemorySize, w));
+                    CK(cudaFuncSetAttribute(fd::ifft_numW_kernel<double, LB, CW>, cudaFuncAttributeMaxDynamicSharedMemorySize, w));
+                });
+                for (int ch : {8, 16, 32}) {
+                    if (LB == 10 && ch == 32) continue;
+                    const int h = (int)fd_smem(ch);
+                    fd_with_bc(f.logB, ch, [&](auto, auto c) {
+                        constexpr int CH = decltype(c)::value;
+                        CK(cudaFuncSetAttribute(fd::fft_h_kernel<LB, CH>, cudaFuncAttributeMaxDynamicSharedMemorySize, h));
+                        CK(cudaFuncSetAttribute(fd::ifft_numH_kernel<LB, CH>, cudaFuncAttributeMaxDynamicSharedMemorySize, h));
+                    });
+                }
+            });
             f.x_dirty = f.w_dirty = f.h_dirty = true;
             f.ok = true;
         }
@@ -451,13 +491,45 @@
     int64_t fd_order(int64_t nblocks) const { static const int o = getenv("CMF_FD_ORDER") ? atoi(getenv("CMF_FD_ORDER")) : 0; return o ? nblocks : 0; }
     int fd_cols_w() const { return fds.B >= 1024 ? 8 : 16; }
     size_t fd_smem(int C) const { return ((size_t)fds.B * (size_t)C + (size_t)fds.B) * sizeof(float2); }
+    void fd_fft_h(__nv_bfloat16 *hi, __nv_bfloat16 *lo, int64_t nb, int V, int full, int64_t t_off) {
+        const int C = fd_cols_h();
+        fd_with_bc(fds.logB, C, [&](auto lb, auto c) {
+            fd::fft_h_kernel<decltype(lb)::value, decltype(c)::value><<<(unsigned)(nb * (fds.Kq / 2 / C)), fd::NT, fd_smem(C), stream>>>(
+                H, hi, lo, K, Tl, Tl + (L - 1), V, nb, full, t_off, fds.Kq, fd_order(nb), fds.tw.p);
+        });
+    }
+    void fd_ifft_numH(const float *Of, float *out, int64_t nb, int V, int64_t nblkp_) {
+        const int C = fd_cols_h();
+        fd_with_bc(fds.logB, C, [&](auto lb, auto c) {
+            fd::ifft_numH_kernel<decltype(lb)::value, decltype(c)::value><<<(unsigned)(nb * (fds.Kq / 2 / C)), fd::NT, fd_smem(C), stream>>>(
+                Of, out, K, Tl, V, nblkp_, fds.Kq, fd_order(nb), fds.tw.p);
+        });
+    }
+    void fd_fft_w(const float *src, __nv_bfloat16 *hi, __nv_bfloat16 *lo, int64_t Nw, int64_t Lw, int64_t ldw, int64_t coff, int xmode) {
+        const int C = fd_cols_w();
+        fd_with_bc(fds.logB, C, [&](auto lb, auto c) {
+            fd::fft_w_kernel<decltype(lb)::value, decltype(c)::value><<<dim3((unsigned)cdiv(Nw, 2 * C), (unsigned)K), fd::NT, fd_smem(C), stream>>>(
+                src, hi, lo, Nw, K, Lw, ldw, coff, xmode, fds.Kq, fds.tw.p);
+        });
+    }
+    template <typename OutT>
+    void fd_ifft_numW(const float *Df, OutT *out, int64_t Nw, int64_t ldi) {
+        const int C = fd_cols_w();
+        fd_with_bc(fds.logB, C, [&](auto lb, auto c) {
+            fd::ifft_numW_kernel<OutT, decltype(lb)::value, decltype(c)::value><<<dim3((unsigned)cdiv(Nw, 2 * C), (unsigned)K), fd::NT, fd_smem(C), stream>>>(
+                Df, out, Nw, ldi, K, L, fds.Kq, fds.tw.p);
+        });
+    }
 
     void fd_build_X() {
         if constexpr (std::is_same<S, float>::value) {
             FdState &f = fds;
             if (!f.x_dirty) return;
             dim3 grid((unsigned)(f.nblkp * cdiv(N, 32)));
-            fd::fft_x_kernel<<<grid, fd::NT, fd_smem(16), stream>>>(X.p, f.Xf_hi.p, f.Xf_lo.p, N, Tl + (L - 1), f.B, f.logB, f.V, f.nblkp, fd_order(f.nblkp));
+            fd_with_b(f.logB, [&](auto lb) {
+                fd::fft_x_kernel<decltype(lb)::value><<<grid, fd::NT, fd_smem(16), stream>>>(X.p, f.Xf_hi.p, f.Xf_lo.p, N, Tl + (L - 1), f.V, f.nblkp,
+                                                                                            fd_order(f.nblkp), f.tw.p);
+            });
             post_launch();
             f.x_dirty = false;
         }
@@ -479,17 +551,15 @@
             tc::tc_kernel<tc::TC_FQC><<<grid, tc::THREADS, tc::SMEM_BYTES, stream>>>(f.mAh[0], f.mAh[1], f.mXfMN[0], f.mXfMN[1], q);
             prof_end();
             post_launch();
-            fd::ifft_numW_kernel<float><<<dim3((unsigned)cdiv(N, 2 * fd_cols_w()), (unsigned)K), fd::NT, fd_smem(fd_cols_w()), stream>>>(f.Df.p, numW.p, N, N, K, L, f.B, f.logB, f.Kq, fd_cols_w());
+            fd_ifft_numW(f.Df.p, numW.p, N, N);
             post_launch();
         }
     }
     void fd_denomH() {
         if constexpr (std::is_same<S, float>::value) {
             FdState &f = fds;
-            fd::fft_w_kernel<<<dim3((unsigned)cdiv(K, 2 * fd_cols_w()), (unsigned)K), fd::NT, fd_smem(fd_cols_w()), stream>>>(
-                Cf.p, f.Ac_hi.p, f.Ac_lo.p, K, K, 2 * L - 1, f.B, f.logB, f.MR, f.Kq, 0, f.Kq, fd_cols_w());
-            post_launch();
-            const int C = fd_cols_h();
+            fd_fft_w(Cf.p, f.Ac_hi.p, f.Ac_lo.p, K, 2 * L - 1, f.MR, f.Kq, 0);
+            post_launch();
             fd_denomH_prefetch();
             f.hf2_valid = false;
             tc::Params q = tc_base_params();
@@ -502,8 +572,7 @@
             const unsigned grid = (unsigned)std::min<int64_t>(q.units, tcs.num_sms);
             tc::tc_kernel<tc::TC_FQT><<<grid, tc::THREADS, tc::SMEM_BYTES, stream>>>(f.mAc[0], f.mAc[1], f.mHf2K[0], f.mHf2K[1], q);
             post_launch();
-            fd::ifft_numH_kernel<<<(unsigned)(f.nblk2 * (f.Kq / 2 / C)), fd::NT, fd_smem(C), stream>>>(
-                f.Of.p, denH.p, K, Tl, f.B, f.logB, f.V2, f.nblk2, C, f.Kq, fd_order(f.nblk2));
+            fd_ifft_numH(f.Of.p, denH.p, f.nblk2, f.V2, f.nblk2);
             post_launch();
         }
     }
@@ -511,9 +580,7 @@
         if constexpr (std::is_same<S, float>::value) {
             FdState &f = fds;
             if (!fd_active() || f.hf2_valid) return;
-            const int C = fd_cols_h();
-            fd::fft_h_kernel<<<(unsigned)(f.nblk2 * (f.Kq / 2 / C)), fd::NT, fd_smem(C), stream>>>(
-                H, f.Hf_hi.p, f.Hf_lo.p, K, Tl, Tl + (L - 1), f.B, f.logB, f.V2, f.nblk2, C, 1, -(L - 1), f.Kq, fd_order(f.nblk2));
+            fd_fft_h(f.Hf_hi.p, f.Hf_lo.p, f.nblk2, f.V2, 1, -(L - 1));
             post_launch();
             f.hf2_valid = true;
         }
@@ -545,13 +612,11 @@
             const size_t need_lp = (size_t)(f.nblk * ntile32);
             if (loss_part.n < need_lp) loss_part.alloc(std::max<size_t>(need_lp, 4096));
             if (f.wx_dirty) {
-                fd::fft_w_kernel<<<dim3((unsigned)cdiv(N, 2 * fd_cols_w()), (unsigned)K), fd::NT, fd_smem(fd_cols_w()), stream>>>(Wi.p, f.Awm_hi.p, f.Awm_lo.p, N, K, L, f.B, f.logB, 2 * N, N, 1, f.Kq, fd_cols_w());
+                fd_fft_w(Wi.p, f.Awm_hi.p, f.Awm_lo.p, N, L, 2 * N, N, 1);
                 post_launch();
                 f.wx_dirty = false;
             }
-            const int C = fd_cols_h();
-            fd::fft_h_kernel<<<(unsigned)(f.nblk * (f.Kq / 2 / C)), fd::NT, fd_smem(C), stream>>>(
-                H, f.Hf_hi.p, f.Hf_lo.p, K, Tl, Tl + (L - 1), f.B, f.logB, f.V, f.nblk, C, 1, -(L - 1), f.Kq, fd_order(f.nblk));
+            fd_fft_h(f.Hf_hi.p, f.Hf_lo.p, f.nblk, f.V, 1, -(L - 1));
             post_launch();
             prof_begin(PROF_CONV);
             for (int64_t b0 = 0; b0 < f.nblk; b0 += f.nbc) {
@@ -567,8 +632,10 @@
                 const unsigned grid = (unsigned)std::min<int64_t>(q.units, tcs.num_sms);
                 tc::tc_kernel<tc::TC_FQX><<<grid, tc::THREADS, tc::SMEM_BYTES, stream>>>(f.mAwm[0], f.mAwm[1], f.mHcK[0], f.mHcK[1], q);
                 post_launch();
-                fd::ifft_resid_kernel<<<(unsigned)(cur * ntile32), fd::NT, fd_smem(16), stream>>>(
-                    f.Yf.p, X.p, loss_part.p + b0 * ntile32, N, Tl, L, f.B, f.logB, f.V, cur, b0, fd_order(cur));
+                fd_with_b(f.logB, [&](auto lb) {
+                    fd::ifft_resid_kernel<decltype(lb)::value><<<(unsigned)(cur * ntile32), fd::NT, fd_smem(16), stream>>>(
+                        f.Yf.p, X.p, loss_part.p + b0 * ntile32, N, Tl, L, f.V, cur, b0, fd_order(cur), f.tw.p);
+                });
                 post_launch();
             }
             prof_end();
@@ -580,9 +647,7 @@
         if constexpr (std::is_same<S, float>::value) {
             FdState &f = fds;
             if (!f.h_dirty) return;
-            const int C = fd_cols_h();
-            fd::fft_h_kernel<<<(unsigned)(f.nblkp * (f.Kq / 2 / C)), fd::NT, fd_smem(C), stream>>>(
-                H, f.Ah_hi.p, f.Ah_lo.p, K, Tl, Tl + (L - 1), f.B, f.logB, f.V, f.nblkp, C, 0, 0, f.Kq, fd_order(f.nblkp));
+            fd_fft_h(f.Ah_hi.p, f.Ah_lo.p, f.nblkp, f.V, 0, 0);
             post_launch();
             f.h_dirty = false;
         }
@@ -592,9 +657,7 @@
             FdState &f = fds;
             f.hf2_valid = false;
             fd_spectrum_H();
-            const int C = fd_cols_h();
-            fd::fft_h_kernel<<<(unsigned)(f.nblkp * (f.Kq / 2 / C)), fd::NT, fd_smem(C), stream>>>(
-                H, f.Hf_hi.p, f.Hf_lo.p, K, Tl, Tl + (L - 1), f.B, f.logB, f.V, f.nblkp, C, 1, 0, f.Kq, fd_order(f.nblkp));
+            fd_fft_h(f.Hf_hi.p, f.Hf_lo.p, f.nblkp, f.V, 1, 0);
             post_launch();
             tc::Params q = tc_base_params();
             q.nprod = 3;
@@ -606,7 +669,7 @@
             const unsigned grid = (unsigned)std::min<int64_t>(q.units, tcs.num_sms);
             tc::tc_kernel<tc::TC_FQC><<<grid, tc::THREADS, tc::SMEM_BYTES, stream>>>(f.mAh[0], f.mAh[1], f.mHfMN[0], f.mHfMN[1], q);
             post_launch();
-            fd::ifft_numW_kernel<double><<<dim3((unsigned)cdiv(K, 2 * fd_cols_w()), (unsigned)K), fd::NT, fd_smem(fd_cols_w()), stream>>>(f.Gf.p, exch1.p, K, f.Kq, K, L, f.B, f.logB, f.Kq, fd_cols_w());
+            fd_ifft_numW(f.Gf.p, exch1.p, K, f.Kq);
             post_launch();
         }
     }
@@ -615,7 +678,7 @@
             FdState &f = fds;
             fd_build_X();
             if (f.w_dirty) {
-                fd::fft_w_kernel<<<dim3((unsigned)cdiv(N, 2 * fd_cols_w()), (unsigned)K), fd::NT, fd_smem(fd_cols_w()), stream>>>(Wi.p, f.Aw_hi.p, f.Aw_lo.p, N, K, L, f.B, f.logB, 2 * N, N, 0, f.Kq, fd_cols_w());
+                fd_fft_w(Wi.p, f.Aw_hi.p, f.Aw_lo.p, N, L, 2 * N, N, 0);
                 post_launch();
                 f.w_dirty = false;
             }
@@ -631,9 +694,7 @@
             tc::tc_kernel<tc::TC_FQT><<<grid, tc::THREADS, tc::SMEM_BYTES, stream>>>(f.mAw[0], f.mAw[1], f.mXfK[0], f.mXfK[1], q);
             prof_end();
             post_launch();
-            const int C = fd_cols_h();
-            fd::ifft_numH_kernel<<<(unsigned)(f.nblk * (f.Kq / 2 / C)), fd::NT, fd_smem(C), stream>>>(
-                f.Of.p, numH.p, K, Tl, f.B, f.logB, f.V, f.nblkp, C, f.Kq, fd_order(f.nblk));
+            fd_ifft_numH(f.Of.p, numH.p, f.nblk, f.V, f.nblkp);
             post_launch();
         }
     }
diff --git a/cmf.jl_b200/csrc/kernels_fd.cuh b/cmf.jl_b200/csrc/kernels_fd.cuh
--- a/cmf.jl_b200/csrc/kernels_fd.cuh
+++ b/cmf.jl_b200/csrc/kernels_fd.cuh
@@ -13,199 +13,242 @@
 constexpr int NT = 512;
 constexpr int KQ_MAX = 128;
 
-__device__ __forceinline__ void make_twiddles(float2 *tw, int B) {
-    for (int m = threadIdx.x; m < B; m += NT) {
+__device__ __forceinline__ float2 add2(float2 a, float2 b) { return __fadd2_rn(a, b); }
+__device__ __forceinline__ float2 sub2(float2 a, float2 b) { return __fadd2_rn(a, make_float2(-b.x, -b.y)); }
+__device__ __forceinline__ float2 mul2(float2 a, float2 b) { return __fmul2_rn(a, b); }
+__device__ __forceinline__ float2 fma2(float2 a, float2 b, float2 c) { return __ffma2_rn(a, b, c); }
+__device__ __forceinline__ float2 bcast(float x) { return make_float2(x, x); }
+
+__global__ void twiddle_kernel(float2 *__restrict__ tw, int B) {
+    const int m = blockIdx.x * blockDim.x + threadIdx.x;
+    if (m < B) {
         float s, c;
         sincospif(-2.0f * (float)m / (float)B, &s, &c);
         tw[m] = make_float2(c, s);
     }
 }
-
-__device__ __forceinline__ int rev(int x, int logB) { return (int)(__brev((unsigned)x) >> (32 - logB)); }
-
-__device__ __forceinline__ float2 cmul(float2 a, float2 w) { return make_float2(a.x * w.x - a.y * w.y, a.x * w.y + a.y * w.x); }
-__device__ __forceinline__ float2 cadd(float2 a, float2 b) { return make_float2(a.x + b.x, a.y + b.y); }
-__device__ __forceinline__ float2 csub(float2 a, float2 b) { return make_float2(a.x - b.x, a.y - b.y); }
+template <int B>
+__device__ __forceinline__ void load_twiddles(float2 *tw, const float2 *__restrict__ twg) {
+#pragma unroll
+    for (int m = threadIdx.x; m < B; m += NT) tw[m] = twg[m];
+}
+
+__device__ __forceinline__ void grid_block_tile(int64_t nbx, int ny, int &blk, int &tile) {
+    const unsigned dv = nbx ? (unsigned)nbx : (unsigned)ny, q = blockIdx.x / dv, r = blockIdx.x - q * dv;
+    blk = (int)(nbx ? r : q);
+    tile = (int)(nbx ? q : r);
+}
+
+template <int LOGB> __device__ __forceinline__ int rev(int x) { return (int)(__brev((unsigned)x) >> (32 - LOGB)); }
+
+template <bool INV> __device__ __forceinline__ float2 twmul(float2 a, float2 w) {
+    const float2 t = mul2(make_float2(a.y, a.x), INV ? make_float2(w.y, -w.y) : make_float2(-w.y, w.y));
+    return fma2(a, bcast(w.x), t);
+}
 template <bool INV> __device__ __forceinline__ float2 mul_mi(float2 a) { return INV ? make_float2(-a.y, a.x) : make_float2(a.y, -a.x); }
-template <bool INV> __device__ __forceinline__ float2 mul_w8(float2 a) {
-    const float r = 0.70710678118654752f;
-    return INV ? make_float2((a.x - a.y) * r, (a.x + a.y) * r) : make_float2((a.x + a.y) * r, (a.y - a.x) * r);
-}
-template <bool INV> __device__ __forceinline__ float2 mul_w83(float2 a) {
-    const float r = 0.70710678118654752f;
-    return INV ? make_float2((-a.x - a.y) * r, (a.x - a.y) * r) : make_float2((a.y - a.x) * r, (-a.x - a.y) * r);
-}
-
-template <bool INV>
-__device__ __forceinline__ void fft_passes(float2 *d, const float2 *tw, int B, int logB, int C) {
-    const int c = threadIdx.x % C, j0 = threadIdx.x / C, jstep = NT / C;
-    int s = 0;
-    for (; s + 2 < logB; s += 3) {
-        const int lq = logB - s - 3, q = 1 << lq, qC = q * C;
-        for (int j = j0; j < (B >> 3); j += jstep) {
+template <bool INV> __device__ __forceinline__ float2 w8_sum(float2 a) {
+    return INV ? add2(make_float2(a.x, a.x), make_float2(-a.y, a.y)) : add2(a, make_float2(a.y, -a.x));
+}
+template <bool INV> __device__ __forceinline__ float2 w83_sum(float2 a) {
+    return INV ? add2(make_float2(-a.x, a.x), make_float2(-a.y, -a.y)) : add2(make_float2(a.y, -a.x), make_float2(-a.x, -a.y));
+}
+
+template <bool INV, int LOGB, int C>
+__device__ __forceinline__ void fft_passes(float2 *d, const float2 *tw) {
+    constexpr int B = 1 << LOGB, JSTEP = NT / C;
+    const float2 rr = bcast(0.70710678118654752f);
+    const int c = threadIdx.x % C, j0 = threadIdx.x / C;
+#pragma unroll
+    for (int s = 0; s + 2 < LOGB; s += 3) {
+        const int lq = LOGB - s - 3, q = 1 << lq, qC = q * C;
+#pragma unroll 1
+        for (int jj = 0; jj < (B / 8 + JSTEP - 1) / JSTEP; ++jj) {
+            const int j = j0 + jj * JSTEP;
+            if ((B / 8) % JSTEP != 0 && j >= B / 8) break;
             const int pos = j & (q - 1), g = j >> lq;
             float2 *r = d + ((g << (lq + 3)) + pos) * C + c;
             float2 a0 = r[0], a1 = r[qC], a2 = r[2 * qC], a3 = r[3 * qC], a4 = r[4 * qC], a5 = r[5 * qC], a6 = r[6 * qC], a7 = r[7 * qC];
-            float2 t;
-            t = csub(a0, a4); a0 = cadd(a0, a4); a4 = t;
-            t = csub(a1, a5); a1 = cadd(a1, a5); a5 = mul_w8<INV>(t);
-            t = csub(a2, a6); a2 = cadd(a2, a6); a6 = mul_mi<INV>(t);
-            t = csub(a3, a7); a3 = cadd(a3, a7); a7 = mul_w83<INV>(t);
-            t = csub(a0, a2); a0 = cadd(a0, a2); a2 = t;
-            t = csub(a1, a3); a1 = cadd(a1, a3); a3 = mul_mi<INV>(t);
-            t = csub(a4, a6); a4 = cadd(a4, a6); a6 = t;
-            t = csub(a5, a7); a5 = cadd(a5, a7); a7 = mul_mi<INV>(t);
-            t = csub(a0, a1); a0 = cadd(a0, a1); a1 = t;
-            t = csub(a2, a3); a2 = cadd(a2, a3); a3 = t;
-            t = csub(a4, a5); a4 = cadd(a4, a5); a5 = t;
-            t = csub(a6, a7); a6 = cadd(a6, a7); a7 = t;
+            float2 t, u5, v7;
+            t = sub2(a0, a4); a0 = add2(a0, a4); a4 = t;
+            t = sub2(a1, a5); a1 = add2(a1, a5); u5 = w8_sum<INV>(t);
+            t = sub2(a2, a6); a2 = add2(a2, a6); a6 = mul_mi<INV>(t);
+            t = sub2(a3, a7); a3 = add2(a3, a7); v7 = mul2(w83_sum<INV>(t), rr);
+            t = sub2(a0, a2); a0 = add2(a0, a2); a2 = t;
+            t = sub2(a1, a3); a1 = add2(a1, a3); a3 = mul_mi<INV>(t);
+            t = sub2(a4, a6); a4 = add2(a4, a6); a6 = t;
+            t = fma2(u5, rr, make_float2(-v7.x, -v7.y)); a5 = fma2(u5, rr, v7); a7 = mul_mi<INV>(t);
+            t = sub2(a0, a1); a0 = add2(a0, a1); a1 = t;
+            t = sub2(a2, a3); a2 = add2(a2, a3); a3 = t;
+            t = sub2(a4, a5); a4 = add2(a4, a5); a5 = t;
+            t = sub2(a6, a7); a6 = add2(a6, a7); a7 = t;
             if (lq > 0) {
                 const int e = pos << s;
-                float2 w;
-#define CMF_TW(m_, a_) w = tw[(m_) * e]; if (INV) w.y = -w.y; a_ = cmul(a_, w);
-                CMF_TW(4, a1) CMF_TW(2, a2) CMF_TW(6, a3) CMF_TW(1, a4) CMF_TW(5, a5) CMF_TW(3, a6) CMF_TW(7, a7)
-#undef CMF_TW
+                a1 = twmul<INV>(a1, tw[4 * e]); a2 = twmul<INV>(a2, tw[2 * e]); a3 = twmul<INV>(a3, tw[6 * e]);
+                a4 = twmul<INV>(a4, tw[e]);     a5 = twmul<INV>(a5, tw[5 * e]); a6 = twmul<INV>(a6, tw[3 * e]);
+                a7 = twmul<INV>(a7, tw[7 * e]);
             }
             r[0] = a0; r[qC] = a1; r[2 * qC] = a2; r[3 * qC] = a3; r[4 * qC] = a4; r[5 * qC] = a5; r[6 * qC] = a6; r[7 * qC] = a7;
         }
         __syncthreads();
     }
-    if (logB - s == 2) {
-        for (int j = j0; j < (B >> 2); j += jstep) {
+    if constexpr (LOGB % 3 == 2) {
+#pragma unroll
+        for (int jj = 0; jj < (B / 4 + JSTEP - 1) / JSTEP; ++jj) {
+            const int j = j0 + jj * JSTEP;
+            if ((B / 4) % JSTEP != 0 && j >= B / 4) break;
             float2 *r = d + (4 * j) * C + c;
             float2 a0 = r[0], a1 = r[C], a2 = r[2 * C], a3 = r[3 * C], t;
-            t = csub(a0, a2); a0 = cadd(a0, a2); a2 = t;
-            t = csub(a1, a3); a1 = cadd(a1, a3); a3 = mul_mi<INV>(t);
-            r[0] = cadd(a0, a1); r[C] = csub(a0, a1); r[2 * C] = cadd(a2, a3); r[3 * C] = csub(a2, a3);
+            t = sub2(a0, a2); a0 = add2(a0, a2); a2 = t;
+            t = sub2(a1, a3); a1 = add2(a1, a3); a3 = mul_mi<INV>(t);
+            r[0] = add2(a0, a1); r[C] = sub2(a0, a1); r[2 * C] = add2(a2, a3); r[3 * C] = sub2(a2, a3);
         }
         __syncthreads();
-    } else if (logB - s == 1) {
-        for (int j = j0; j < (B >> 1); j += jstep) {
+    } else if constexpr (LOGB % 3 == 1) {
+#pragma unroll
+        for (int jj = 0; jj < (B / 2 + JSTEP - 1) / JSTEP; ++jj) {
+            const int j = j0 + jj * JSTEP;
+            if ((B / 2) % JSTEP != 0 && j >= B / 2) break;
             float2 *r0 = d + (2 * j) * C + c, *r1 = r0 + C;
             const float2 a = *r0, b = *r1;
-            *r0 = cadd(a, b);
-            *r1 = csub(a, b);
+            *r0 = add2(a, b);
+            *r1 = sub2(a, b);
         }
         __syncthreads();
     }
 }
 
-__device__ __forceinline__ void unpack_pair(const float2 *d, int f, int B, int logB, int C, int p, float &ar, float &ai, float &br,
-                                            float &bi) {
-    const float2 z = d[rev(f, logB) * C + p], y = d[rev((B - f) & (B - 1), logB) * C + p];
-    ar = 0.5f * (z.x + y.x); ai = 0.5f * (z.y - y.y);
-    br = 0.5f * (z.y + y.y); bi = -0.5f * (z.x - y.x);
-}
-
-__device__ __forceinline__ void pack_pair(float2 *d, int f, int B, int C, int p, float2 re, float2 im) {
+template <int LOGB, int C>
+__device__ __forceinline__ void unpack_pair(const float2 *d, int f, int p, float2 &re, float2 &im) {
+    constexpr int B = 1 << LOGB;
+    const float2 z = d[rev<LOGB>(f) * C + p], y = d[rev<LOGB>((B - f) & (B - 1)) * C + p];
+    const float2 sm = add2(z, y), df = sub2(z, y);
+    re = mul2(sm, bcast(0.5f));
+    im = mul2(make_float2(df.y, df.x), make_float2(0.5f, -0.5f));
+}
+
+template <int LOGB, int C>
+__device__ __forceinline__ void pack_pair(float2 *d, int f, int p, float2 re, float2 im) {
+    constexpr int B = 1 << LOGB;
     if (f == 0 || f == B / 2) im = make_float2(0.f, 0.f);
-    d[f * C + p] = make_float2(re.x - im.y, im.x + re.y);
-    if (f > 0 && f < B / 2) d[(B - f) * C + p] = make_float2(re.x + im.y, re.y - im.x);
-}
-
-__device__ __forceinline__ void split2(float a, float b, uint32_t &h, uint32_t &l) {
-    const __nv_bfloat162 hh = __floats2bfloat162_rn(a, b);
-    const float2 hf = __bfloat1622float2(hh);
-    const __nv_bfloat162 ll = __floats2bfloat162_rn(a - hf.x, b - hf.y);
+    const float2 v = make_float2(im.y, im.x);
+    const float2 sm = add2(re, v), df = sub2(re, v);
+    d[f * C + p] = make_float2(df.x, sm.y);
+    if (f > 0 && f < B / 2) d[(B - f) * C + p] = make_float2(sm.x, df.y);
+}
+
+__device__ __forceinline__ void split2(float2 ab, uint32_t &h, uint32_t &l) {
+    const __nv_bfloat162 hh = __floats2bfloat162_rn(ab.x, ab.y);
+    const float2 lf = sub2(ab, __bfloat1622float2(hh));
+    const __nv_bfloat162 ll = __floats2bfloat162_rn(lf.x, lf.y);
     h = *reinterpret_cast<const uint32_t *>(&hh);
     l = *reinterpret_cast<const uint32_t *>(&ll);
 }
-__device__ __forceinline__ void store_split2(__nv_bfloat16 *hi, __nv_bfloat16 *lo, int64_t idx, float a, float b) {
+__device__ __forceinline__ void store_split2(__nv_bfloat16 *hi, __nv_bfloat16 *lo, int64_t idx, float2 ab) {
     uint32_t h, l;
-    split2(a, b, h, l);
+    split2(ab, h, l);
     *reinterpret_cast<uint32_t *>(hi + idx) = h;
     *reinterpret_cast<uint32_t *>(lo + idx) = l;
 }
 
+template <int LOGB>
 __global__ void __launch_bounds__(NT, CMF_FD_MINB)
 fft_x_kernel(const float *__restrict__ X, __nv_bfloat16 *__restrict__ hi, __nv_bfloat16 *__restrict__ lo, int64_t N, int64_t xcols,
-             int B, int logB, int V, int64_t nblkp, int64_t nbx) {
-    extern __shared__ float2 fd_smem[];
-    constexpr int C = 16;
-    float2 *d = fd_smem, *tw = fd_smem + (size_t)B * C;
-    const int ny = (int)((N + 31) / 32);
-    const int64_t b = nbx ? blockIdx.x % nbx : blockIdx.x / ny;
-    const int p = threadIdx.x % C;
-    const int64_t n = (int64_t)(nbx ? blockIdx.x / nbx : blockIdx.x % ny) * 32 + 2 * p;
-    make_twiddles(tw, B);
-    {
-        const int i0 = threadIdx.x / C, istep = NT / C;
-        const int64_t lim64 = xcols - b * V;
+             int V, int64_t nblkp, int64_t nbx, const float2 *__restrict__ twg) {
+    constexpr int B = 1 << LOGB, C = 16, ISTEP = NT / C;
+    extern __shared__ float2 fd_smem[];
+    float2 *d = fd_smem, *tw = fd_smem + B * C;
+    int b, tile;
+    grid_block_tile(nbx, (int)((N + 31) / 32), b, tile);
+    const int p = threadIdx.x % C;
+    const int n = tile * 32 + 2 * p;
+    load_twiddles<B>(tw, twg);
+    {
+        const int i0 = threadIdx.x / C;
+        const int64_t lim64 = xcols - (int64_t)b * V;
         const int lim = (n < N) ? (int)(lim64 < 0 ? 0 : (lim64 > B ? B : lim64)) : 0;
-        const float *src = X + (b * V + i0) * N + n;
-        for (int i = i0; i < B; i += LD_U * istep, src += (int64_t)LD_U * istep * N) {
+        const float *src = X + ((int64_t)b * V + i0) * N + n;
+        float2 *dst = d + i0 * C + p;
+#pragma unroll 1
+        for (int i = i0; i < B; i += LD_U * ISTEP, src += (int64_t)LD_U * ISTEP * N, dst += LD_U * ISTEP * C) {
             float2 v[LD_U];
 #pragma unroll
             for (int u = 0; u < LD_U; ++u) {
                 v[u] = make_float2(0.f, 0.f);
-                if (i + u * istep < lim) v[u] = *reinterpret_cast<const float2 *>(src + (int64_t)u * istep * N);
+                if (i + u * ISTEP < lim) v[u] = *reinterpret_cast<const float2 *>(src + (int64_t)u * ISTEP * N);
             }
 #pragma unroll
             for (int u = 0; u < LD_U; ++u)
-                if (i + u * istep < B) d[(i + u * istep) * C + p] = v[u];
-        }
-    }
-    __syncthreads();
-    fft_passes<false>(d, tw, B, logB, C);
+                if (B % (LD_U * ISTEP) == 0 || i + u * ISTEP < B) dst[u * ISTEP * C] = v[u];
+        }
+    }
+    __syncthreads();
+    fft_passes<false, LOGB, C>(d, tw);
     if (n >= N) return;
     for (int f = threadIdx.x / C; f <= B / 2; f += NT / C) {
-        float ar, ai, br, bi;
-        unpack_pair(d, f, B, logB, C, p, ar, ai, br, bi);
+        float2 re, im;
+        unpack_pair<LOGB, C>(d, f, p, re, im);
         const int64_t r = ((int64_t)f * nblkp + b) * 2;
-        store_split2(hi, lo, r * N + n, ar, br);
-        store_split2(hi, lo, (r + 1) * N + n, ai, bi);
-    }
-}
-
+        store_split2(hi, lo, r * N + n, re);
+        store_split2(hi, lo, (r + 1) * N + n, im);
+    }
+}
+
+template <int LOGB, int C>
 __global__ void __launch_bounds__(NT, CMF_FD_MINB)
 fft_h_kernel(const float *__restrict__ H, __nv_bfloat16 *__restrict__ hi, __nv_bfloat16 *__restrict__ lo, int64_t K, int64_t Tl,
-             int64_t hcols, int B, int logB, int V, int64_t nblkp, int C, int full, int64_t t_off, int kq, int64_t nbx) {
+             int64_t hcols, int V, int64_t nblkp, int full, int64_t t_off, int kq, int64_t nbx,
+             const float2 *__restrict__ twg) {
+    constexpr int B = 1 << LOGB, ISTEP = NT / C;
     const int64_t KQ = kq, MROWS = 2 * kq;
     extern __shared__ float2 fd_smem[];
-    float2 *d = fd_smem, *tw = fd_smem + (size_t)B * C;
-    const int ny = (kq / 2) / C;
-    const int64_t b = nbx ? blockIdx.x % nbx : blockIdx.x / ny;
-    const int p = threadIdx.x % C;
-    const int k = 2 * ((int)(nbx ? blockIdx.x / nbx : blockIdx.x % ny) * C + p);
-    make_twiddles(tw, B);
-    {
-        const int i0 = threadIdx.x / C, istep = NT / C;
+    float2 *d = fd_smem, *tw = fd_smem + B * C;
+    int bi, tile;
+    grid_block_tile(nbx, (kq / 2) / C, bi, tile);
+    const int64_t b = bi;
+    const int p = threadIdx.x % C;
+    const int k = 2 * (tile * C + p);
+    load_twiddles<B>(tw, twg);
+    {
+        const int i0 = threadIdx.x / C;
         const int64_t tb = b * V + t_off;
         const int64_t lim64 = full ? (hcols - tb) : ((Tl - tb < V) ? Tl - tb : V);
         const int lim = (int)(lim64 < 0 ? 0 : (lim64 > B ? B : lim64));
         const float *src = H + (tb + i0) * K + k;
+        float2 *dst = d + i0 * C + p;
         const bool pair = ((K & 1) == 0) && (k + 1 < K);
-        for (int i = i0; i < B; i += LD_U * istep, src += (int64_t)LD_U * istep * K) {
+#pragma unroll 1
+        for (int i = i0; i < B; i += LD_U * ISTEP, src += (int64_t)LD_U * ISTEP * K, dst += LD_U * ISTEP * C) {
             float2 v[LD_U];
 #pragma unroll
             for (int u = 0; u < LD_U; ++u) {
                 v[u] = make_float2(0.f, 0.f);
-                if (i + u * istep < lim) {
-                    const float *q = src + (int64_t)u * istep * K;
+                if (i + u * ISTEP < lim) {
+                    const float *q = src + (int64_t)u * ISTEP * K;
                     if (pair) v[u] = *reinterpret_cast<const float2 *>(q);
                     else { if (k < K) v[u].x = q[0]; if (k + 1 < K) v[u].y = q[1]; }
                 }
             }
 #pragma unroll
             for (int u = 0; u < LD_U; ++u)
-                if (i + u * istep < B) d[(i + u * istep) * C + p] = v[u];
-        }
-    }
-    __syncthreads();
-    fft_passes<false>(d, tw, B, logB, C);
-    for (int f = threadIdx.x / C; f <= B / 2; f += NT / C) {
-        float ar, ai, br, bi;
-        unpack_pair(d, f, B, logB, C, p, ar, ai, br, bi);
+                if (B % (LD_U * ISTEP) == 0 || i + u * ISTEP < B) dst[u * ISTEP * C] = v[u];
+        }
+    }
+    __syncthreads();
+    fft_passes<false, LOGB, C>(d, tw);
+    const int64_t rs = full ? 2 * KQ : 2 * MROWS;
+    const int64_t rstep = (int64_t)(NT / C) * nblkp * rs;
+    int64_t r = ((int64_t)(threadIdx.x / C) * nblkp + b) * rs + k;
+    for (int f = threadIdx.x / C; f <= B / 2; f += NT / C, r += rstep) {
+        float2 re, im;
+        unpack_pair<LOGB, C>(d, f, p, re, im);
         uint32_t hr, lr, hi_, li_;
-        split2(ar, br, hr, lr);
-        split2(ai, bi, hi_, li_);
+        split2(re, hr, lr);
+        split2(im, hi_, li_);
         if (full) {
-            const int64_t r = (((int64_t)f * nblkp + b) * 2) * KQ + k;
             *reinterpret_cast<uint32_t *>(hi + r) = hr; *reinterpret_cast<uint32_t *>(lo + r) = lr;
             *reinterpret_cast<uint32_t *>(hi + r + KQ) = hi_; *reinterpret_cast<uint32_t *>(lo + r + KQ) = li_;
             continue;
         }
-        const int64_t r = (((int64_t)f * nblkp + b) * 2) * MROWS + k;
         const uint32_t sg = 0x80008000u;
         *reinterpret_cast<uint32_t *>(hi + r) = hr; *reinterpret_cast<uint32_t *>(lo + r) = lr;
         *reinterpret_cast<uint32_t *>(hi + r + KQ) = hi_ ^ sg; *reinterpret_cast<uint32_t *>(lo + r + KQ) = li_ ^ sg;
@@ -214,152 +257,167 @@
     }
 }
 
+template <int LOGB, int C>
 __global__ void __launch_bounds__(NT, CMF_FD_MINB)
 fft_w_kernel(const float *__restrict__ Wi, __nv_bfloat16 *__restrict__ hi, __nv_bfloat16 *__restrict__ lo, int64_t N, int64_t K,
-             int64_t L, int B, int logB, int64_t ldw, int64_t coff, int xmode, int kq, int C) {
+             int64_t L, int64_t ldw, int64_t coff, int xmode, int kq, const float2 *__restrict__ twg) {
+    constexpr int B = 1 << LOGB, ISTEP = NT / C;
     const int64_t KQ = kq, MROWS = 2 * kq;
     extern __shared__ float2 fd_smem[];
-    float2 *d = fd_smem, *tw = fd_smem + (size_t)B * C;
+    float2 *d = fd_smem, *tw = fd_smem + B * C;
     const int64_t k = blockIdx.y;
     const int p = threadIdx.x % C;
     const int64_t n = (int64_t)blockIdx.x * (2 * C) + 2 * p;
-    make_twiddles(tw, B);
-    {
-        const int i0 = threadIdx.x / C, istep = NT / C;
-        for (int i = i0; i < B; i += LD_U * istep) {
+    load_twiddles<B>(tw, twg);
+    {
+        const int i0 = threadIdx.x / C;
+        const float *src = Wi + ((int64_t)i0 * K + k) * N + n;
+        float2 *dst = d + i0 * C + p;
+#pragma unroll 1
+        for (int i = i0; i < B; i += LD_U * ISTEP, src += (int64_t)LD_U * ISTEP * K * N, dst += LD_U * ISTEP * C) {
             float2 v[LD_U];
 #pragma unroll
             for (int u = 0; u < LD_U; ++u) {
-                const int ii = i + u * istep;
+                const int ii = i + u * ISTEP;
                 v[u] = make_float2(0.f, 0.f);
                 if (ii < L && n < N) {
-                    const float *src = Wi + ((int64_t)ii * K + k) * N + n;
-                    if ((N & 1) == 0) v[u] = *reinterpret_cast<const float2 *>(src);
-                    else { v[u].x = src[0]; if (n + 1 < N) v[u].y = src[1]; }
+                    const float *q = src + (int64_t)u * ISTEP * K * N;
+                    if ((N & 1) == 0) v[u] = *reinterpret_cast<const float2 *>(q);
+                    else { v[u].x = q[0]; if (n + 1 < N) v[u].y = q[1]; }
                 }
             }
 #pragma unroll
             for (int u = 0; u < LD_U; ++u)
-                if (i + u * istep < B) d[(i + u * istep) * C + p] = v[u];
-        }
-    }
-    __syncthreads();
-    fft_passes<false>(d, tw, B, logB, C);
+                if (B % (LD_U * ISTEP) == 0 || i + u * ISTEP < B) dst[u * ISTEP * C] = v[u];
+        }
+    }
+    __syncthreads();
+    fft_passes<false, LOGB, C>(d, tw);
     if (n >= N) return;
     for (int f = threadIdx.x / C; f <= B / 2; f += NT / C) {
-        float ar, ai, br, bi;
-        unpack_pair(d, f, B, logB, C, p, ar, ai, br, bi);
+        float2 re, im;
+        unpack_pair<LOGB, C>(d, f, p, re, im);
+        const float2 nim = make_float2(-im.x, -im.y);
         if (xmode) {
-            const int64_t r0 = (((int64_t)f * 2 + 0) * MROWS + k) * N + n, r1 = (((int64_t)f * 2 + 1) * MROWS + k) * N + n;
-            store_split2(hi, lo, r0, ar, br);
-            store_split2(hi, lo, r0 + KQ * N, -ai, -bi);
-            store_split2(hi, lo, r1, ai, bi);
-            store_split2(hi, lo, r1 + KQ * N, ar, br);
+            const int64_t r0 = (((int64_t)f * 2 + 0) * MROWS + k) * N + n, r1 = r0 + MROWS * N;
+            store_split2(hi, lo, r0, re);
+            store_split2(hi, lo, r0 + KQ * N, nim);
+            store_split2(hi, lo, r1, im);
+            store_split2(hi, lo, r1 + KQ * N, re);
             continue;
         }
-        const int64_t re = ((int64_t)f * MROWS + k) * ldw, im = ((int64_t)f * MROWS + KQ + k) * ldw;
-        store_split2(hi, lo, re + n, ar, br);
-        store_split2(hi, lo, re + coff + n, ai, bi);
-        store_split2(hi, lo, im + n, -ai, -bi);
-        store_split2(hi, lo, im + coff + n, ar, br);
-    }
-}
-
-__global__ void __launch_bounds__(NT, CMF_FD_MINB)
-ifft_numH_kernel(const float *__restrict__ Of, float *__restrict__ numH, int64_t K, int64_t Tl, int B, int logB, int V,
-                 int64_t nblkp, int C, int kq, int64_t nbx) {
+        const int64_t rw = ((int64_t)f * MROWS + k) * ldw + n, iw = rw + KQ * ldw;
+        store_split2(hi, lo, rw, re);
+        store_split2(hi, lo, rw + coff, im);
+        store_split2(hi, lo, iw, nim);
+        store_split2(hi, lo, iw + coff, re);
+    }
+}
+
+template <int LOGB, int C>
+__global__ void __launch_bounds__(NT, CMF_FD_MINB)
+ifft_numH_kernel(const float *__restrict__ Of, float *__restrict__ numH, int64_t K, int64_t Tl, int V, int64_t nblkp, int kq,
+                 int64_t nbx, const float2 *__restrict__ twg) {
+    constexpr int B = 1 << LOGB, FSTEP = NT / C;
     const int64_t KQ = kq, MROWS = 2 * kq;
     extern __shared__ float2 fd_smem[];
-    float2 *d = fd_smem, *tw = fd_smem + (size_t)B * C;
-    const int ny = (kq / 2) / C;
-    const int64_t b = nbx ? blockIdx.x % nbx : blockIdx.x / ny;
-    const int p = threadIdx.x % C;
-    const int k = 2 * ((int)(nbx ? blockIdx.x / nbx : blockIdx.x % ny) * C + p);
-    make_twiddles(tw, B);
-    {
-        const int f0 = threadIdx.x / C, fstep = NT / C;
+    float2 *d = fd_smem, *tw = fd_smem + B * C;
+    int bi, tile;
+    grid_block_tile(nbx, (kq / 2) / C, bi, tile);
+    const int64_t b = bi;
+    const int p = threadIdx.x % C;
+    const int k = 2 * (tile * C + p);
+    load_twiddles<B>(tw, twg);
+    {
+        const int f0 = threadIdx.x / C;
+        const int64_t ustep = (int64_t)FSTEP * nblkp * MROWS;
         const float *o = Of + ((int64_t)f0 * nblkp + b) * MROWS + k;
-        for (int f = f0; f <= B / 2; f += 4 * fstep, o += (int64_t)4 * fstep * nblkp * MROWS) {
+#pragma unroll 1
+        for (int f = f0; f <= B / 2; f += 4 * FSTEP, o += 4 * ustep) {
             float2 re[4], im[4];
 #pragma unroll
             for (int u = 0; u < 4; ++u)
-                if (f + u * fstep <= B / 2) {
-                    const float *q = o + (int64_t)u * fstep * nblkp * MROWS;
+                if (f + u * FSTEP <= B / 2) {
+                    const float *q = o + u * ustep;
                     re[u] = *reinterpret_cast<const float2 *>(q); im[u] = *reinterpret_cast<const float2 *>(q + KQ);
                 }
 #pragma unroll
             for (int u = 0; u < 4; ++u)
-                if (f + u * fstep <= B / 2) pack_pair(d, f + u * fstep, B, C, p, re[u], im[u]);
-        }
-    }
-    __syncthreads();
-    fft_passes<true>(d, tw, B, logB, C);
-    const float sc = 1.0f / (float)B;
+                if (f + u * FSTEP <= B / 2) pack_pair<LOGB, C>(d, f + u * FSTEP, p, re[u], im[u]);
+        }
+    }
+    __syncthreads();
+    fft_passes<true, LOGB, C>(d, tw);
+    const float2 sc = bcast(1.0f / (float)B);
     const bool pair = ((K & 1) == 0) && (k + 1 < K);
     for (int i = threadIdx.x / C; i < V; i += NT / C) {
         const int64_t t = b * V + i;
         if (t >= Tl) break;
-        const float2 z = d[rev(i, logB) * C + p];
-        if (pair) *reinterpret_cast<float2 *>(numH + t * K + k) = make_float2(z.x * sc, z.y * sc);
-        else { if (k < K) numH[t * K + k] = z.x * sc; if (k + 1 < K) numH[t * K + k + 1] = z.y * sc; }
-    }
-}
-
+        const float2 z = mul2(d[rev<LOGB>(i) * C + p], sc);
+        if (pair) *reinterpret_cast<float2 *>(numH + t * K + k) = z;
+        else { if (k < K) numH[t * K + k] = z.x; if (k + 1 < K) numH[t * K + k + 1] = z.y; }
+    }
+}
+
+template <int LOGB>
 __global__ void __launch_bounds__(NT, CMF_FD_MINB)
 ifft_resid_kernel(const float *__restrict__ Yf, const float *__restrict__ X, double *__restrict__ partial, int64_t N, int64_t Tl,
-                  int64_t L, int B, int logB, int V, int64_t nbc, int64_t b0, int64_t nbx) {
+                  int64_t L, int V, int64_t nbc, int64_t b0, int64_t nbx, const float2 *__restrict__ twg) {
+    constexpr int B = 1 << LOGB, C = 16, FSTEP = NT / C, ISTEP = NT / C;
     extern __shared__ float2 fd_smem[];
     __shared__ double red[NT / 32];
-    constexpr int C = 16;
-    float2 *d = fd_smem, *tw = fd_smem + (size_t)B * C;
+    float2 *d = fd_smem, *tw = fd_smem + B * C;
     const int ny = (int)((N + 31) / 32);
-    const int64_t bc = nbx ? blockIdx.x % nbx : blockIdx.x / ny;
-    const int by = (int)(nbx ? blockIdx.x / nbx : blockIdx.x % ny);
-    const int p = threadIdx.x % C;
-    const int64_t n = (int64_t)by * 32 + 2 * p;
-    make_twiddles(tw, B);
-    {
-        const int f0 = threadIdx.x / C, fstep = NT / C;
+    int bc, by;
+    grid_block_tile(nbx, ny, bc, by);
+    const int p = threadIdx.x % C;
+    const int n = by * 32 + 2 * p;
+    load_twiddles<B>(tw, twg);
+    {
+        const int f0 = threadIdx.x / C;
+        const int64_t ustep = (int64_t)FSTEP * nbc * 2 * N;
         const float *y = Yf + (((int64_t)f0 * nbc + bc) * 2) * N + n;
-        for (int f = f0; f <= B / 2; f += 4 * fstep, y += (int64_t)4 * fstep * nbc * 2 * N) {
+#pragma unroll 1
+        for (int f = f0; f <= B / 2; f += 4 * FSTEP, y += 4 * ustep) {
             float2 re[4], im[4];
 #pragma unroll
             for (int u = 0; u < 4; ++u) {
                 re[u] = make_float2(0.f, 0.f); im[u] = re[u];
-                if (f + u * fstep <= B / 2 && n < N) {
-                    const float *q = y + (int64_t)u * fstep * nbc * 2 * N;
+                if (f + u * FSTEP <= B / 2 && n < N) {
+                    const float *q = y + u * ustep;
                     re[u] = *reinterpret_cast<const float2 *>(q); im[u] = *reinterpret_cast<const float2 *>(q + N);
                 }
             }
 #pragma unroll
             for (int u = 0; u < 4; ++u)
-                if (f + u * fstep <= B / 2) pack_pair(d, f + u * fstep, B, C, p, re[u], im[u]);
-        }
-    }
-    __syncthreads();
-    fft_passes<true>(d, tw, B, logB, C);
-    const float sc = 1.0f / (float)B;
+                if (f + u * FSTEP <= B / 2) pack_pair<LOGB, C>(d, f + u * FSTEP, p, re[u], im[u]);
+        }
+    }
+    __syncthreads();
+    fft_passes<true, LOGB, C>(d, tw);
+    const float2 sc = bcast(1.0f / (float)B);
     double accd = 0.0;
     if (n < N) {
-        const int istep = NT / C;
-        const int64_t tb = (b0 + bc) * V - (L - 1);
-        for (int i = (int)(L - 1) + threadIdx.x / C; i < B; i += LD_U * istep) {
+        const int64_t tb = (b0 + bc) * (int64_t)V - (L - 1);
+        const int lim = (int)(Tl - tb < B ? Tl - tb : B);
+        const int i0 = (int)(L - 1) + threadIdx.x / C;
+        const float *xs = X + (tb + i0) * N + n;
+#pragma unroll 1
+        for (int i = i0; i < B; i += LD_U * ISTEP, xs += (int64_t)LD_U * ISTEP * N) {
             float2 x[LD_U];
 #pragma unroll
             for (int u = 0; u < LD_U; ++u) {
-                const int ii = i + u * istep;
                 x[u] = make_float2(0.f, 0.f);
-                if (ii < B && tb + ii < Tl) x[u] = *reinterpret_cast<const float2 *>(X + (tb + ii) * N + n);
+                if (i + u * ISTEP < lim) x[u] = *reinterpret_cast<const float2 *>(xs + (int64_t)u * ISTEP * N);
             }
             float acc = 0.f;
 #pragma unroll
             for (int u = 0; u < LD_U; ++u) {
-                const int ii = i + u * istep;
-                if (ii < B && tb + ii < Tl) {
-                    const float2 z = d[rev(ii, logB) * C + p];
-                    const float r0 = z.x * sc - x[u].x, r1 = z.y * sc - x[u].y;
-                    acc = fmaf(r0, r0, acc);
-                    acc = fmaf(r1, r1, acc);
+                const int ii = i + u * ISTEP;
+                if (ii < lim) {
+                    const float2 r = fma2(d[rev<LOGB>(ii) * C + p], sc, make_float2(-x[u].x, -x[u].y));
+                    acc = fmaf(r.x, r.x, acc);
+                    acc = fmaf(r.y, r.y, acc);
                 }
             }
             accd += (double)acc;
@@ -372,54 +430,57 @@
     if (threadIdx.x == 0) {
         double s = 0.0;
         for (int w = 0; w < NT / 32; ++w) s += red[w];
-        partial[bc * ny + by] = s;
-    }
-}
-
-template <typename OutT>
-__global__ void __launch_bounds__(NT, CMF_FD_MINB)
-ifft_numW_kernel(const float *__restrict__ Df, OutT *__restrict__ out, int64_t N, int64_t ldi, int64_t K, int64_t L, int B, int logB,
-                 int kq, int C) {
+        partial[(int64_t)bc * ny + by] = s;
+    }
+}
+
+template <typename OutT, int LOGB, int C>
+__global__ void __launch_bounds__(NT, CMF_FD_MINB)
+ifft_numW_kernel(const float *__restrict__ Df, OutT *__restrict__ out, int64_t N, int64_t ldi, int64_t K, int64_t L, int kq,
+                 const float2 *__restrict__ twg) {
+    constexpr int B = 1 << LOGB, FSTEP = NT / C;
     const int64_t KQ = kq, MROWS = 2 * kq;
     extern __shared__ float2 fd_smem[];
-    float2 *d = fd_smem, *tw = fd_smem + (size_t)B * C;
+    float2 *d = fd_smem, *tw = fd_smem + B * C;
     const int64_t k = blockIdx.y;
     const int p = threadIdx.x % C;
     const int64_t n = (int64_t)blockIdx.x * (2 * C) + 2 * p;
-    make_twiddles(tw, B);
-    {
-        const int f0 = threadIdx.x / C, fstep = NT / C;
-        for (int f = f0; f <= B / 2; f += 4 * fstep) {
+    load_twiddles<B>(tw, twg);
+    {
+        const int f0 = threadIdx.x / C;
+        const int64_t ustep = (int64_t)FSTEP * MROWS * ldi;
+        const float *src = Df + ((int64_t)f0 * MROWS + k) * ldi + n;
+#pragma unroll 1
+        for (int f = f0; f <= B / 2; f += 4 * FSTEP, src += 4 * ustep) {
             float2 re[4], im[4];
 #pragma unroll
             for (int u = 0; u < 4; ++u) {
-                const int ff = f + u * fstep;
                 re[u] = make_float2(0.f, 0.f); im[u] = re[u];
-                if (ff <= B / 2 && n < N) {
-                    re[u] = *reinterpret_cast<const float2 *>(Df + ((int64_t)ff * MROWS + k) * ldi + n);
-                    im[u] = *reinterpret_cast<const float2 *>(Df + ((int64_t)ff * MROWS + KQ + k) * ldi + n);
+                if (f + u * FSTEP <= B / 2 && n < N) {
+                    re[u] = *reinterpret_cast<const float2 *>(src + u * ustep);
+                    im[u] = *reinterpret_cast<const float2 *>(src + u * ustep + KQ * ldi);
                 }
             }
 #pragma unroll
             for (int u = 0; u < 4; ++u)
-                if (f + u * fstep <= B / 2) pack_pair(d, f + u * fstep, B, C, p, re[u], im[u]);
-        }
-    }
-    __syncthreads();
-    fft_passes<true>(d, tw, B, logB, C);
+                if (f + u * FSTEP <= B / 2) pack_pair<LOGB, C>(d, f + u * FSTEP, p, re[u], im[u]);
+        }
+    }
+    __syncthreads();
+    fft_passes<true, LOGB, C>(d, tw);
     if (n >= N) return;
-    const float sc = 1.0f / (float)B;
+    const float2 sc = bcast(1.0f / (float)B);
     for (int l = threadIdx.x / C; l < L; l += NT / C) {
-        const float2 z = d[rev(l, logB) * C + p];
+        const float2 z = mul2(d[rev<LOGB>(l) * C + p], sc);
         OutT *o = out + ((int64_t)l * K + k) * N + n;
         if (sizeof(OutT) == 4) {
-            *reinterpret_cast<float2 *>(o) = make_float2(z.x * sc, z.y * sc);
+            *reinterpret_cast<float2 *>(o) = z;
         } else {
-            o[0] = (OutT)(z.x * sc);
-            if (n + 1 < N) o[1] = (OutT)(z.y * sc);
-        }
-    }
-}
-
-}
-}
+            o[0] = (OutT)z.x;
+            if (n + 1 < N) o[1] = (OutT)z.y;
+        }
+    }
+}
+
+}
+}
```
